# Martinsos/edlib

Measured on AMD Instinct MI355X. Metric: GCUPS (cell updates/s), 1M x 150bp HW reads vs 5Mb target, higher is better.
Workload: dtype u32

## Files before the change

edlib_amd/csrc/engine.hip:

```cpp
#include "engine.hpp"
#include "flat_results.hpp"
#include <sched.h>

#if defined(__x86_64__)
#include <immintrin.h>
#endif
#include <algorithm>
#include <chrono>
#include <atomic>
#include <cmath>
#include <cstdarg>
#include <cstring>
#include <condition_variable>
#include <mutex>
#include <system_error>
#include <thread>

namespace edlib_amd {


static void build_eq8(std::vector<uint8_t>& eq8, const EdlibEqualityPair* eqs, int neq) {
    eq8.assign(256 * 256, 0);
    for (int a = 0; a < 256; ++a) eq8[a * 256 + a] = 1;
    for (int i = 0; i < neq; ++i) {
// ... 16 lines not shown
        const int miss = _mm_movemask_epi8(_mm_cmpeq_epi8(_mm_and_si128(a, b), zero));
        if (miss) return i + __builtin_ctz((unsigned)miss);
    }
    return i;
}
#endif

void build_tables(Tables& tab, const uint8_t* targets, long long totalTargetBytes,
                         const EdlibEqualityPair* eqs, int neq) {
    memset(tab.presence, 0, sizeof tab.presence);
    memset(tab.tlut, 0, sizeof tab.tlut);
    memset(tab.idToByte, 0, sizeof tab.idToByte);
    bool seen[256] = {false};
    tab.sigmaT = 0;
    uint8_t lo[16] = {0}, hi[16] = {0}; int hiBit[16]; int hiBits = 0; bool nibbleOk = true;
    for (int h = 0; h < 16; ++h) hiBit[h] = -1;
#if defined(__x86_64__)
    static const bool haveSsse3 = __builtin_cpu_supports("ssse3");
#else
    static const bool haveSsse3 = false;
#endif
    long long i = 0;
    while (i < totalTargetBytes) {
#if defined(__x86_64__)
        if (haveSsse3 && nibbleOk && tab.sigmaT > 0) {
            i = first_outside_ssse3(targets, i, totalTargetBytes, lo, hi);
            if (i >= totalTargetBytes) break;
        }
#endif
        const uint8_t b = targets[i++];
        if (!seen[b]) {
            seen[b] = true;
            tab.tlut[b] = (uint8_t)tab.sigmaT;
            tab.idToByte[tab.sigmaT] = b;
            tab.presence[b >> 5] |= 1u << (b & 31);
            ++tab.sigmaT;
            if (hiBit[b >> 4] < 0) { if (hiBits < 8) hiBit[b >> 4] = hiBits++; else nibbleOk = false; }
            if (nibbleOk) { hi[b >> 4] = (uint8_t)(1u << hiBit[b >> 4]); lo[b & 15] |= (uint8_t)(1u << hiBit[b >> 4]); }
        }
    }
    tab.eq8.clear();
    if (neq > 0) build_eq8(tab.eq8, eqs, neq);
    for (int q = 0; q < 256; ++q) {
        uint16_t mask = 0;
        for (int s = 0; s < tab.sigmaT && s < 16; ++s)
            if (tab.eq8.empty() ? (q == tab.idToByte[s]) : (tab.eq8[q * 256 + tab.idToByte[s]] != 0)) mask |= (uint16_t)(1u << s);
        tab.eqtbl[q] = mask;
    }
}


__global__ void __launch_bounds__(256)
alphabet_count_kernel(const uint8_t* __restrict__ qpool, const long long* __restrict__ qoff,
                      const uint8_t* __restrict__ tpool, const long long* __restrict__ toff,
                      int shared, const uint32_t* __restrict__ basePresence,
                      const int* __restrict__ unitIdx, int* __restrict__ out)
{
    __shared__ uint32_t s_seen[256];
    s_seen[threadIdx.x] = 0u;
    __syncthreads();
    const int u = unitIdx[blockIdx.x];
    auto scan = [&](const uint8_t* pool, long long lo, long long hi) {
        for (long long c = (lo >> 4) + threadIdx.x; (c << 4) < hi; c += 256) {
            const uint4 v = *reinterpret_cast<const uint4*>(pool + (c << 4));
            const uint32_t d[4] = {v.x, v.y, v.z, v.w};
            const long long at = c << 4;
            if (at >= lo && at + 16 <= hi) {
#pragma unroll
                for (int k = 0; k < 16; ++k) s_seen[(d[k >> 2] >> (8 * (k & 3))) & 0xffu] = 1u;
            } else {
#pragma unroll
                for (int k = 0; k < 16; ++k)
                    if (at + k >= lo && at + k < hi) s_seen[(d[k >> 2] >> (8 * (k & 3))) & 0xffu] = 1u;
            }
        }
    };
    scan(qpool, qoff[u], qoff[u + 1]);
    if (!shared) scan(tpool, toff[u], toff[u + 1]);
    __syncthreads();
    bool present = s_seen[threadIdx.x] != 0u;
    if (shared) present = present || ((basePresence[threadIdx.x >> 5] >> (threadIdx.x & 31)) & 1u);
    const int n = __syncthreads_count(present ? 1 : 0);
    if (threadIdx.x == 0) out[blockIdx.x] = n;
}

__global__ void __launch_bounds__(256)
alphabet_count_short_kernel(const uint8_t* __restrict__ qpool, const long long* __restrict__ qoff,
                            const uint8_t* __restrict__ tpool, const long long* __restrict__ toff,
                            int shared, const uint32_t* __restrict__ basePresence,
                            const int* __restrict__ unitIdx, int n, int* __restrict__ out)
{
    __shared__ uint32_t s_seen[4][64];
    const int lane = threadIdx.x & 63, wv = threadIdx.x >> 6;
    const int slot = blockIdx.x * 4 + wv;
    if (slot >= n) return;
    uint8_t* const seen = reinterpret_cast<uint8_t*>(s_seen[wv]);
    s_seen[wv][lane] = 0u;
    const int u = unitIdx[slot];
    auto scan = [&](const uint8_t* pool, long long lo, long long hi) {
        for (long long c = (lo >> 4) + lane; (c << 4) < hi; c += 64) {
            const uint4 v = *reinterpret_cast<const uint4*>(pool + (c << 4));
            const uint32_t d[4] = {v.x, v.y, v.z, v.w};
            const long long at = c << 4;
#pragma unroll
            for (int k = 0; k < 16; ++k)
                if (at + k >= lo && at + k < hi) seen[(d[k >> 2] >> (8 * (k & 3))) & 0xffu] = 1;
        }
    };
    scan(qpool, qoff[u], qoff[u + 1]);
    if (!shared) scan(tpool, toff[u], toff[u + 1]);
    __builtin_amdgcn_fence(__ATOMIC_RELEASE, "wavefront");
    __builtin_amdgcn_wave_barrier();
    uint32_t w = s_seen[wv][lane];
    if (shared) {
        const uint32_t bits = (basePresence[lane >> 3] >> (4 * (lane & 7))) & 0xfu;
        w |= (bits & 1u) | ((bits & 2u) << 7) | ((bits & 4u) << 14) | ((bits & 8u) << 21);
    }
    int cnt = ((w & 0xffu) != 0) + ((w & 0xff00u) != 0) + ((w & 0xff0000u) != 0) + ((w & 0xff000000u) != 0);
#pragma unroll
    for (int off = 32; off >= 1; off >>= 1) cnt += __shfl_xor(cnt, off, 64);
    if (lane == 0) out[slot] = cnt;
}


Batch::~Batch() {
    DeviceGuard guard(device_);
    if (side_) { (void)hipStreamSynchronize(side_); pool_stream_release(side_); }
    if (aux_) { (void)hipStreamSynchronize(aux_); (void)hipStreamDestroy(aux_); }
    if (stream_) { (void)hipStreamSynchronize(stream_); pool_stream_release(stream_); }
    wideGateRelease();
    for (auto& p : scanEvents_) { pool_event_release(p.first, device_); pool_event_release(p.second, device_); }
}

int roundup(int x, int q) { return (x + q - 1) / q * q; }

int Batch::init(const char* queries, const long long* qoff, int n, const char* targets,
                const long long* toff, int numTargets, EdlibAlignConfig cfg, int device, bool bothStrands, bool hits)
{
    if (n < 0 || (numTargets != 1 && numTargets != n)) { set_error("bad batch shape"); return 1; }
    if (hits) {
        if (numTargets != 1 || bothStrands) { set_error("hit-list read batch: one shared target, one strand"); return 1; }
        if (cfg.mode != EDLIB_MODE_HW) { set_error("hit-list read batch: config.mode must be EDLIB_MODE_HW (SHW and NW have no hit list)"); return 1; }
        if (cfg.task != EDLIB_TASK_DISTANCE) {
            set_error("hit-list read batch: config.task must be EDLIB_TASK_DISTANCE (start locations and paths: align the chosen windows with a pair batch)");
            return 1;
        }
        if (cfg.k < 0) { set_error("hit-list read batch: config.k must be >= 0 (got %d)", cfg.k); return 1; }
        for (int u = 0; u < n; ++u)
            if (qoff[u + 1] - qoff[u] > 32LL * kMaxReadWords) {
                set_error("hit-list read batch: read %d has %lld bases, the limit is %d", u, qoff[u + 1] - qoff[u], 32 * kMaxReadWords);
                return 1;
            }
        bool seen[256] = {false};
        int sigma = 0;
        for (long long j = toff[0]; j < toff[1]; ++j) if (!seen[(uint8_t)targets[j]]) { seen[(uint8_t)targets[j]] = true; ++sigma; }
        if (sigma > 16) { set_error("hit-list read batch: the target has %d distinct symbols, the limit is 16", sigma); return 1; }
    }
    hits_ = hits;
    if (bothStrands && (numTargets != 1 || n > 0x3fffffff)) { set_error("bad both-strand batch shape"); return 1; }
    if (check_device(device)) return 1;
    keep_config(cfg, cfg_, eqs_);
    device_ = device;
    strands_ = bothStrands;
    shared_ = (numTargets == 1);
    if (copy_offsets(qoff, n, "query", qoff_)) return 1;
    const int numReads = n;
    const long long qb = qoff[0];
    if (strands_) {
        n = 2 * numReads;
        qoff_.resize((size_t)n + 1);
        for (int i = 0; i < numReads; ++i) { qoff_[2 * i] = 2 * (qoff[i] - qb); qoff_[2 * i + 1] = 2 * (qoff[i] - qb) + (qoff[i + 1] - qoff[i]); }
        qoff_[n] = 2 * (qoff[numReads] - qb);
    }
    n_ = n;
    if (copy_offsets(toff, numTargets, "target", toff_)) return 1;
    const long long qbytes = qoff_[n] - qoff_[0], tbytes = toff_[numTargets] - toff_[0];
    build_tables(tab_, reinterpret_cast<const uint8_t*>(targets) + toff_[0], tbytes,
                 eqs_.data(), (int)eqs_.size());

    pool_quarantine(false);
    DeviceGuard guard(device_);
    EDLIB_AMD_HIP(guard.status);
    EDLIB_AMD_HIP(pool_stream(&stream_));
    EDLIB_AMD_HIP(evRun0_.create()); EDLIB_AMD_HIP(evRun1_.create());

    const long long tb = toff_[0];
    if (!strands_) for (auto& v : qoff_) v -= qb;
    for (auto& v : toff_) v -= tb;
    {
        const bool inlineT = qbytes + tbytes <= (1 << 20), inlineQ = inlineT && !strands_;
        size_t at = 0;
        auto take = [&](size_t bytes) { const size_t o = at; at = (at + bytes + 15) & ~(size_t)15; return o; };
        const size_t oQoff = take(qoff_.size() * sizeof(long long)), oToff = take(toff_.size() * sizeof(long long));
        const size_t oTlut = take(256), oId = take(256), oEq4 = take(512), oPres = take(32);
        const size_t oQ = inlineQ ? take((size_t)qbytes + 16) : 0, oT = inlineT ? take((size_t)tbytes + 16) : 0;
        EDLIB_AMD_HIP(d_in_.alloc(at));
        EDLIB_AMD_HIP(h_in_.alloc(at));
        uint8_t* h = h_in_.p;
        memcpy(h + oQoff, qoff_.data(), qoff_.size() * sizeof(long long));
        memcpy(h + oToff, toff_.data(), toff_.size() * sizeof(long long));
        memcpy(h + oTlut, tab_.tlut, 256); memcpy(h + oId, tab_.idToByte, 256);
        memcpy(h + oEq4, tab_.eqtbl, 512); memcpy(h + oPres, tab_.presence, 32);
        d_qoff_.alias(d_in_.p + oQoff, qoff_.size()); d_toff_.alias(d_in_.p + oToff, toff_.size());
        d_tlut_.alias(d_in_.p + oTlut, 256); d_idToByte_.alias(d_in_.p + oId, 256);
        d_eqtbl_.alias(d_in_.p + oEq4, 256); d_presence_.alias(d_in_.p + oPres, 8);
        if (inlineQ) {
            if (qbytes) memcpy(h + oQ, queries + qb, (size_t)qbytes);
            memset(h + oQ + qbytes, 0, 16);
            d_qpool_.alias(d_in_.p + oQ, (size_t)qbytes + 16);
        } else {
            EDLIB_AMD_HIP(d_qpool_.alloc((size_t)qbytes + 16));
            if (qbytes && !strands_) EDLIB_AMD_HIP(hipMemcpy(d_qpool_.p, queries + qb, (size_t)qbytes, hipMemcpyHostToDevice));
        }
        if (inlineT) {
            if (tbytes) memcpy(h + oT, targets + tb, (size_t)tbytes);
            memset(h + oT + tbytes, 0, 16);
            d_tpool_.alias(d_in_.p + oT, (size_t)tbytes + 16);
        } else {
            EDLIB_AMD_HIP(d_tpool_.alloc((size_t)tbytes + 16));
            if (tbytes) EDLIB_AMD_HIP(hipMemcpy(d_tpool_.p, targets + tb, (size_t)tbytes, hipMemcpyHostToDevice));
        }
        EDLIB_AMD_HIP(hipMemcpyAsync(d_in_.p, h, at, hipMemcpyHostToDevice, stream_));
    }
    if (strands_) {
        const size_t inBytes = (size_t)(qbytes / 2);
        DevBuf<uint8_t> d_raw;
        EDLIB_AMD_HIP(d_raw.alloc(inBytes + 16));
        if (inBytes) EDLIB_AMD_HIP(hipMemcpy(d_raw.p, queries + qb, inBytes, hipMemcpyHostToDevice));
        EDLIB_AMD_HIP(hipMemsetAsync(d_qpool_.p, 0, (size_t)qbytes + 16, stream_));
        EDLIB_AMD_HIP(launch_strand_pool(d_raw.p, d_qoff_.p, numReads, d_qpool_.p, stream_));
        EDLIB_AMD_HIP(hipStreamSynchronize(stream_));
        EDLIB_AMD_HIP(h_strand_.alloc(2 * (size_t)numReads));
        memset(h_strand_.p, 0, 2 * (size_t)numReads);
    }

    const int mode = (int)cfg_.mode;
    const int modeIn = (int)cfg.mode;
    const bool readsOk = shared_ && tlen(0) > 0 && (tab_.sigmaT <= 4 || (tab_.sigmaT <= 16 && modeIn == EDLIB_MODE_HW));
    syms_ = peq_syms(tab_.sigmaT);
    banded_ = mode == EDLIB_MODE_HW;
    static const int filterFrom = [] {
        const char* e = getenv("EDLIB_AMD_FILTER");
        if (!e || !e[0]) return kFilterFromWords;
        const int v = atoi(e);
        return v <= 0 ? 0 : std::max(kMaxReadWords + 1, std::min(v, kMaxLongReadWords4 + 1));
    }();
    const bool filter = filterFrom > 0 && readsOk && banded_ && modeIn == EDLIB_MODE_HW;
    int groupWords = kMaxReadWords;
    if (banded_ && modeIn == EDLIB_MODE_HW && syms_ <= 8)
        for (int w : {10, 12, 14, 16, 24, 32})
            if (w <= (syms_ == 4 ? kMaxLongReadWords4 : kMaxLongReadWords) && (!filter || w < filterFrom)) groupWords = w;
    const int maxReadLen = 32 * groupWords;
    std::vector<std::vector<int>> byWords(kMaxLongReadWords4 + 1);
    for (int u = 0; u < n; ++u) {
        const int m = qlen(u), T = tlen(u);
        if (m == 0 || T == 0) emptyUnits_.push_back(u);
        else if (readsOk && m <= maxReadLen) { readUnits_.push_back(u); byWords[read_group_words(m)].push_back(u); }
        else if (filter) longUnits_.push_back(u);
        else pairUnits_.push_back(u);
    }
    stats.cells = 0;
    for (int u = 0; u < n; ++u) stats.cells += (long long)qlen(u) * tlen(u);
    {
        alphaUnits_ = emptyUnits_;
        alphaUnits_.insert(alphaUnits_.end(), pairUnits_.begin(), pairUnits_.end());
        alphaUnits_.insert(alphaUnits_.end(), longUnits_.begin(), longUnits_.end());
        long long total = 0;
        for (int u : alphaUnits_) total += qlen(u) + (shared_ ? 0 : tlen(u));
        alphaOnHost_ = h_in_.p && d_qpool_.p && !d_qpool_.owned && total <= 65536;
        alphaBytes_ = total;
    }

    for (int w = 1; w <= kMaxLongReadWords4; ++w) {
        if (byWords[w].empty()) continue;
        std::unique_ptr<ReadGroup> g;
        if (makeGroup(byWords[w], w, g)) return 1;
        if (strands_) {
            for (int sl = 0; sl < g->nslots; sl += 2)
                if (g->perm[sl] >= 0 && ((g->perm[sl] & 1) || g->perm[sl + 1] != g->perm[sl] + 1)) { set_error("both strands: mates are not in adjacent slots"); return 1; }
            g->mates = true;
            EDLIB_AMD_HIP(g->d_win.alloc((size_t)g->nslots / 2));
        }
        groups_.push_back(std::move(g));
    }
    if (initFlatPairs()) return 1;
    const int T = shared_ ? tlen(0) : 0;
    if (!groups_.empty() || !longUnits_.empty()) {
        EDLIB_AMD_HIP(d_tpk_.alloc((size_t)(T + 15) / 16 + 4));
        EDLIB_AMD_HIP(hipMemsetAsync(d_tpk_.p, 0, d_tpk_.bytes(), stream_));
        EDLIB_AMD_HIP(d_wordSteps_.alloc(1));
        EDLIB_AMD_HIP(d_trows_.alloc(((size_t)(T + 15) / 16 + 2) * 8));
    }
    return 0;
}

int Batch::makeGroup(const std::vector<int>& units, int w, std::unique_ptr<ReadGroup>& g, long long oneRoundWaves)
{
    const int mode = (int)cfg_.mode;
    const int T = shared_ ? tlen(0) : 0;
    g.reset(new ReadGroup);
    g->nwords = w;
    g->nslots = roundup((int)units.size(), 64);
    g->perm.assign(g->nslots, -1);
    g->mMin = 0x7fffffff;
    for (int u : units) g->mMin = std::min(g->mMin, qlen(u));
    std::copy(units.begin(), units.end(), g->perm.begin());
    const int nrblk = g->nslots / 64;
    if (mode == EDLIB_MODE_HW) {
        const long long wantWaves = 131072;
        g->warm = 2 * 32 * w - 1;
        long long S = (wantWaves + nrblk - 1) / nrblk;
        const long long maxS = std::max<long long>(1, std::min<long long>(std::min(65535, std::max(1, T / 4096)), T / (4LL * g->warm)));
        S = std::max(1LL, std::min(S, maxS));
        if (oneRoundWaves > 0 && oneRoundWaves / nrblk >= 1) S = std::min(S, oneRoundWaves / nrblk);
        g->segLen = roundup((int)((T + S - 1) / S), 16);
        g->numSegments = (T + g->segLen - 1) / g->segLen;
    } else {
        g->numSegments = 1; g->segLen = roundup(T, 16); g->warm = 0;
    }
    const size_t ns = (size_t)g->nslots, S = (size_t)g->numSegments;
    EDLIB_AMD_HIP(g->d_perm.alloc(ns));
    EDLIB_AMD_HIP(hipMemcpyAsync(g->d_perm.p, g->perm.data(), ns * sizeof(int), hipMemcpyHostToDevice, stream_));
    EDLIB_AMD_HIP(g->d_qlen.alloc(ns)); EDLIB_AMD_HIP(g->d_kinit.alloc(ns));
    g->zeroCopy = ns <= 1024 && pool_enabled();
    if (g->zeroCopy) {
        EDLIB_AMD_HIP(g->hostOut.alloc((ns * 20 + ns + 1) * sizeof(int)));
        int* h = reinterpret_cast<int*>(g->hostOut.p);
        memset(h, 0, (ns * 20 + ns + 1) * sizeof(int));
        g->d_best.alias(h, ns); g->d_total.alias(h + ns, ns); g->d_alphaExtra.alias(h + 2 * ns, ns);
        g->d_flags.alias(h + 3 * ns, ns + 1); g->d_pos.alias(h + 4 * ns + 1, ns * 16);
    } else
    EDLIB_AMD_HIP(g->d_alphaExtra.alloc(ns));
    EDLIB_AMD_HIP(g->d_peq.alloc(ns * (size_t)syms_ * w));
    EDLIB_AMD_HIP(g->d_segBest.alloc(ns * S)); EDLIB_AMD_HIP(g->d_segCnt.alloc(ns * S));
    EDLIB_AMD_HIP(g->d_segPos.alloc(ns * S * 8));
    if (!g->zeroCopy) {
        EDLIB_AMD_HIP(g->d_best.alloc(ns)); EDLIB_AMD_HIP(g->d_total.alloc(ns));
        EDLIB_AMD_HIP(g->d_pos.alloc(ns * 16)); EDLIB_AMD_HIP(g->d_flags.alloc(ns + 1));
    }
    return 0;
}

hipError_t Batch::uploadEq8() {
    if (tab_.eq8.empty() || d_eq8_.p) return hipSuccess;
    hipError_t e = d_eq8_.alloc(65536);
    if (e != hipSuccess) return e;
    return hipMemcpyAsync(d_eq8_.p, tab_.eq8.data(), 65536, hipMemcpyHostToDevice, stream_);
}


void Batch::scanTimerStart() {
    if (scanEventsUsed_ == scanEvents_.size()) {
        hipEvent_t a = nullptr, b = nullptr; int dev = 0;
        (void)pool_event(&a, &dev); (void)pool_event(&b, &dev);
        scanEvents_.push_back({a, b});
    }
    (void)hipEventRecord(scanEvents_[scanEventsUsed_].first, stream_);
}
void Batch::scanTimerStop() {
    (void)hipEventRecord(scanEvents_[scanEventsUsed_].second, stream_);
    ++scanEventsUsed_;
    ++stats.scan_launches;
}


void finalize_semiglobal(UnitResult& r, int kcfg, int m, int best, const int* pos, long long npos) {
    const int W = ((m + 63) / 64) * 64 - m;
    const bool kAllowsM = (kcfg < 0 || kcfg >= m);
    r.ends.clear();
    if (best < 0) {
        if (W > 0 && kAllowsM) { r.editDistance = m; r.ends.push_back(-1); r.hasEnds = true; }
        else { r.editDistance = -1; r.hasEnds = false; }
        return;
    }
    r.editDistance = best;
    r.hasEnds = true;
    if (W > 0 && best == m) r.ends.push_back(-1);
    r.ends.append(pos, (size_t)npos);
}

void blank_record(UnitResult& r) {
    r.status = EDLIB_STATUS_OK; r.editDistance = -1; r.alphabetLength = 0;
    r.hasEnds = r.hasStarts = r.hasAlignment = false;
    r.ends.clear(); r.starts.clear(); r.opsView = nullptr; r.opsViewLen = 0;
}

void finalize_global(UnitResult& r, int kcfg, int mode, int T, int score) {
    if (kcfg >= 0 && score > kcfg) { r.editDistance = -1; r.hasEnds = false; return; }
    r.editDistance = score;
    if (mode == EDLIB_MODE_NW) { r.hasEnds = true; r.ends.assign(1, T - 1); }
    else r.hasEnds = false;
}

int Batch::alphabetBuffers()
{
    const size_t n = alphaUnits_.size();
    if (!side_) EDLIB_AMD_HIP(pool_stream(&side_));
    EDLIB_AMD_HIP(evA_.create());
    if (!d_alphaIdx_.p) {
        EDLIB_AMD_HIP(d_alphaIdx_.alloc(n)); EDLIB_AMD_HIP(d_alphaOut_.alloc(n)); EDLIB_AMD_HIP(alphaPin_.alloc(n * sizeof(int)));
        EDLIB_AMD_HIP(hipMemcpyAsync(d_alphaIdx_.p, alphaUnits_.data(), n * sizeof(int), hipMemcpyHostToDevice, side_));
    }
    return 0;
}

int Batch::alphabetLengthsBegin(hipEvent_t after)
{
    alphaPending_ = false;
    if (alphaUnits_.empty() || alphaOnHost_) return 0;
    const size_t n = alphaUnits_.size();
    if (alphabetBuffers()) return 1;
    EDLIB_AMD_HIP(hipEventRecord(evA_.e, stream_));
    EDLIB_AMD_HIP(hipStreamWaitEvent(side_, evA_.e, 0));
    if (after) EDLIB_AMD_HIP(hipStreamWaitEvent(side_, after, 0));
    if (alphaBytes_ <= 4096LL * (long long)n)
        hipLaunchKernelGGL(alphabet_count_short_kernel, dim3((unsigned)((n + 3) / 4)), dim3(256), 0, side_,
                           d_qpool_.p, d_qoff_.p, d_tpool_.p, d_toff_.p, shared_ ? 1 : 0, d_presence_.p,
                           d_alphaIdx_.p, (int)n, d_alphaOut_.p);
    else
    hipLaunchKernelGGL(alphabet_count_kernel, dim3((unsigned)n), dim3(256), 0, side_,
                       d_qpool_.p, d_qoff_.p, d_tpool_.p, d_toff_.p, shared_ ? 1 : 0, d_presence_.p,
                       d_alphaIdx_.p, d_alphaOut_.p);
    EDLIB_AMD_HIP(hipGetLastError());
    EDLIB_AMD_HIP(evB_.create());
    EDLIB_AMD_HIP(hipEventRecord(evB_.e, side_));
    EDLIB_AMD_HIP(hipMemcpyAsync(alphaPin_.p, d_alphaOut_.p, n * sizeof(int), hipMemcpyDeviceToHost, side_));
    alphaPending_ = true;
    return 0;
}

int Batch::alphabetLengthsEnd(std::vector<UnitResult>& res)
{
    if (alphaUnits_.empty()) return 0;
    if (alphaOnHost_) {
        const uint8_t* hq = h_in_.p + (d_qpool_.p - d_in_.p);
        const uint8_t* ht = h_in_.p + (d_tpool_.p - d_in_.p);
        for (int u : alphaUnits_) {
            bool seen[256] = {false};
            int cnt = 0;
            auto add = [&](const uint8_t* p, long long len) { for (long long i = 0; i < len; ++i) if (!seen[p[i]]) { seen[p[i]] = true; ++cnt; } };
            add(hq + qoff_[u], qlen(u));
            if (!shared_) add(ht + toff_[u], tlen(u));
            else for (int b = 0; b < 256; ++b) if ((tab_.presence[b >> 5] >> (b & 31)) & 1u) { if (!seen[b]) { seen[b] = true; ++cnt; } }
            res[u].alphabetLength = cnt;
        }
        return 0;
    }
    if (!alphaPending_) return 0;
    EDLIB_AMD_HIP(hipStreamSynchronize(side_));
    alphaPending_ = false;
    const int* out = reinterpret_cast<const int*>(alphaPin_.p);
    for (size_t i = 0; i < alphaUnits_.size(); ++i) res[alphaUnits_[i]].alphabetLength = out[i];
    return 0;
}



int Batch::run()
{
    const int rc = runImpl();
    if (rc && wideGateHeld_) {
        if (stream_) { DeviceGuard guard(device_); (void)hipStreamSynchronize(stream_); (void)hipGetLastError(); }
        wideGateRelease();
    }
    return rc;
}

int Batch::beginRun(hipError_t guardStatus)
{
    EDLIB_AMD_HIP(guardStatus);
    const long long cells = stats.cells;
    stats = EdlibAmdBatchStats{};
    stats.cells = cells;
    scanEventsUsed_ = 0;
    wordStepsPending_ = false;
    EDLIB_AMD_HIP(hipEventRecord(evRun0_.e, stream_));
    return 0;
}

int Batch::enqueueWordSteps()
{
    EDLIB_AMD_HIP(h_wordSteps_.alloc(sizeof(unsigned long long)));
    EDLIB_AMD_HIP(hipMemcpyAsync(h_wordSteps_.p, d_wordSteps_.p, sizeof(unsigned long long), hipMemcpyDeviceToHost, stream_));
    wordStepsPending_ = true;
    return 0;
}

int Batch::endRun()
{
    EDLIB_AMD_HIP(hipEventRecord(evRun1_.e, stream_));
    EDLIB_AMD_HIP(hipStreamSynchronize(stream_));
    float ms = 0;
    EDLIB_AMD_HIP(hipEventElapsedTime(&ms, evRun0_.e, evRun1_.e));
    stats.run_ms = ms;
    if (wordStepsPending_) { stats.word_steps += (long long)*reinterpret_cast<unsigned long long*>(h_wordSteps_.p); wordStepsPending_ = false; }
    for (size_t i = 0; i < scanEventsUsed_; ++i) {
        float t = 0;
        EDLIB_AMD_HIP(hipEventElapsedTime(&t, scanEvents_[i].first, scanEvents_[i].second));
        stats.scan_ms += t;
    }
    return 0;
}

int Batch::runImpl()
{
    pool_quarantine(false);
    Lap lap;
    DeviceGuard guard(device_);
    haveResults_ = hitsHaveRun_ = hitList_.result.fetched = false;
    if (beginRun(guard.status)) return 1;
    if (hits_) return runReadHits();
    hostStrandCounts_[0] = hostStrandCounts_[1] = hostStrandCounts_[2] = hostStrandCounts_[3] = 0;
    opsKeep_.clear();
    knownSplits_.clear();
    wideGateRelease();
    wideSerial_ = false;
    viewReady_ = false; cigar_[0].ready = cigar_[1].ready = false; lastRunFlat_ = false;
    opsOwned_.clear();
    std::vector<UnitResult>& res = work_;
    resetRecords(res);
    if (d_ringSteps_.p) EDLIB_AMD_HIP(hipMemsetAsync(d_ringSteps_.p, 0, sizeof(unsigned long long), stream_));
    ringStepsUsed_ = false;
    lap("run: reset records");
    answerEmptyUnits(res);
    alphaDeferred_ = !flatPairs_ && cfg_.mode == EDLIB_MODE_NW && cfg_.task == EDLIB_TASK_DISTANCE && pairUnits_.size() >= 8192 &&
                     groups_.empty() && longUnits_.empty();
    if (!alphaDeferred_ && alphabetLengthsBegin()) return 1;
    flatDone_ = false;
    if (flatPairs_ && runFlatPhase(res, lap)) return 1;
    if (packTarget()) return 1;
    if (runReads()) return 1;
    readsCollected_ = groups_.empty();
    lap("run: reads scans");
    if (!readsCollected_ && cfg_.task != EDLIB_TASK_DISTANCE && collectReads(res)) return 1;
    lap("run: collect reads");
    pairNow_ = pairUnits_;
    if (!longUnits_.empty() && runLongReads(res, lap)) return 1;
    if (banded_ && (!groups_.empty() || !longUnits_.empty()) && enqueueWordSteps()) return 1;
    if (flatDone_) pairNow_.clear();
    if (!pairNow_.empty() && runPairPhase(res, lap)) return 1;
    lap("run: finalize pairs");
    if (!flatDone_ && alphabetLengthsEnd(res)) return 1;
    lap("run: phase 1 (distance)");
    if (strands_ && !res.empty() && resolveStrandsOnHost(res)) return 1;
    live_.clear();
    const bool laterPhases = !flatDone_ && (cfg_.task == EDLIB_TASK_LOC || cfg_.task == EDLIB_TASK_PATH);
    if (laterPhases)
        for (int u = 0; u < n_; ++u)
            if (qlen(u) > 0 && tlen(u) > 0 && res[u].editDistance >= 0) live_.push_back(u);
    if (laterPhases && runStartsPhase(res, lap)) return 1;
    lap("run: phase 2 (starts)");
    if (cfg_.task == EDLIB_TASK_PATH && runPathsPhase(res, lap)) return 1;
    lap("run: phase 3 (paths)");
    if (ringStepsUsed_) EDLIB_AMD_HIP(hipMemcpyAsync(h_ringSteps_.p, d_ringSteps_.p, sizeof(unsigned long long), hipMemcpyDeviceToHost, stream_));
    if (endRun()) return 1;
    if (ringStepsUsed_) stats.word_steps += (long long)*reinterpret_cast<unsigned long long*>(h_ringSteps_.p);
    startStats();
    results_.swap(res);
    haveResults_ = true;
    lap("run: stats");
    if (strands_ && lap.on) {
        int c[4];
        if (strandCounts(c)) return 1;
        fprintf(stderr, "[edlib_amd] strands: %d reads, forward %d, reverse %d, both %d, none %d, located %zu\n", outN(), c[0], c[1],
                c[2], c[3], laterPhases ? live_.size() : (size_t)0);
    }
    return 0;
}

void Batch::resetRecords(std::vector<UnitResult>& res)
{
    const bool lazy = (cfg_.task == EDLIB_TASK_DISTANCE && pairUnits_.empty() && longUnits_.empty() && emptyUnits_.empty() && !groups_.empty()) || flatPairs_;
    pairsCollected_ = true;
    deferReset_ = false;
    deferReadsReset_ = false;
    if (lazy) { res.clear(); return; }
    const size_t keep = std::min(res.size(), (size_t)n_);
    res.resize((size_t)n_);
    deferReset_ = emptyUnits_.empty() && groups_.empty() && longUnits_.empty() && !flatPairs_ && pairUnits_.size() == (size_t)n_;
    deferReadsReset_ = !deferReset_ && cfg_.task != EDLIB_TASK_DISTANCE && emptyUnits_.empty() && pairUnits_.empty() &&
                       longUnits_.empty() && !flatPairs_ && readUnits_.size() == (size_t)n_;
    if (!deferReset_ && !deferReadsReset_) for (size_t u = 0; u < keep; ++u) blank_record(res[u]);
}

void Batch::answerEmptyUnits(std::vector<UnitResult>& res)
{
    const int mode = (int)cfg_.mode;
    for (int u : emptyUnits_) {
        UnitResult& r = res[u];
        const int m = qlen(u), T = tlen(u);
        if (mode == EDLIB_MODE_NW) { r.editDistance = std::max(m, T); r.ends.assign(1, T - 1); r.hasEnds = true; }
        else if (mode == EDLIB_MODE_SHW || mode == EDLIB_MODE_HW) { r.editDistance = m; r.ends.assign(1, -1); r.hasEnds = true; }
        else r.status = EDLIB_STATUS_ERROR;
    }
}

int Batch::runFlatPhase(std::vector<UnitResult>& res, Lap& lap)
{
    bool fell = false;
    if (runPairsFlat(fell)) return 1;
    if (fell) {
        res.resize((size_t)n_);
        for (size_t u = 0; u < res.size(); ++u) blank_record(res[u]);
    } else { flatDone_ = true; pairsCollected_ = false; lastRunFlat_ = true; }
    lap("run: flat pairs");
    return 0;
}

// ... 471 lines not shown
```

edlib_amd/csrc/engine.hpp:

```cpp
#pragma once
#include "../../include/edlib_amd.h"
#include "common.hpp"
#include "pair_kernels.hpp"
#include "lanepair.hpp"
#include "reads_kernels.hpp"
#include "cross_kernels.hpp"
#include "window_kernels.hpp"
#include "strands.hpp"

#include <chrono>
#include <deque>
#include <functional>
#include <memory>
#include <vector>

namespace edlib_amd {

struct Tables {
    uint8_t tlut[256];
    uint8_t idToByte[256];
    int sigmaT = 0;
    uint32_t presence[8];
    uint16_t eqtbl[256];
    std::vector<uint8_t> eq8;
};

struct UnitSpec {
    long long qoff; int qlen; int qstep;
    long long toff; int tlen; int tstep;
    int kinit;
    int skip = 0;
    int band = 0;
};

struct SolveOut {
    std::vector<int> score, count, last;
    std::vector<long long> posStart;
    std::vector<int> posFlat;
    std::vector<const uint8_t*> opsPtr;
    std::vector<int> opsLen;
    std::vector<std::shared_ptr<PinBuf>> opsBufs;
    void reset(size_t n) {
        score.assign(n, -1); count.assign(n, 0); last.assign(n, -1);
        posStart.assign(n + 1, 0); posFlat.clear();
        opsPtr.assign(n, nullptr); opsLen.assign(n, 0); opsBufs.clear();
    }
};

struct Assembler {
    struct Pick { const SolveOut* from = nullptr; size_t q = 0; };
    std::vector<Pick> pick;
    explicit Assembler(size_t n) : pick(n) {}
    void take(size_t i, const SolveOut& from, size_t q) { pick[i].from = &from; pick[i].q = q; }
    void write(SolveOut& out) const {
        out.reset(pick.size());
        for (size_t i = 0; i < pick.size(); ++i) {
            if (const SolveOut* p = pick[i].from) {
                const size_t q = pick[i].q;
                out.score[i] = p->score[q]; out.count[i] = p->count[q]; out.last[i] = p->last[q];
                out.posFlat.insert(out.posFlat.end(), p->posFlat.begin() + p->posStart[q], p->posFlat.begin() + p->posStart[q + 1]);
            }
            out.posStart[i + 1] = (long long)out.posFlat.size();
        }
    }
};

struct BandLadder {
    int mode;
    bool (*enter)(const UnitSpec& u, long long& K);
    UnitSpec (*level)(const UnitSpec& u, long long K);
    bool (*final)(const UnitSpec& u, const UnitSpec& level, int score);
};

struct OpsOut {
    const uint8_t* p = nullptr;
    int len = 0;
    std::vector<uint8_t> own;
};

class LocList {
public:
    LocList() = default;
    ~LocList() { delete big_; }
    LocList(const LocList& o) { append(o.data(), o.n_); }
    LocList& operator=(const LocList& o) { if (this != &o) { clear(); append(o.data(), o.n_); } return *this; }
    LocList(LocList&& o) noexcept : n_(o.n_), big_(o.big_) { in_[0] = o.in_[0]; in_[1] = o.in_[1]; o.n_ = 0; o.big_ = nullptr; }
    LocList& operator=(LocList&& o) noexcept {
        if (this != &o) { delete big_; n_ = o.n_; big_ = o.big_; in_[0] = o.in_[0]; in_[1] = o.in_[1]; o.n_ = 0; o.big_ = nullptr; }
        return *this;
    }
    size_t size() const { return n_; }
    bool empty() const { return n_ == 0; }
    const int* data() const { return n_ <= kInline ? in_ : big_->data(); }
    int* data() { return n_ <= kInline ? in_ : big_->data(); }
    int operator[](size_t i) const { return data()[i]; }
    int& operator[](size_t i) { return data()[i]; }
    void clear() { n_ = 0; }
    void push_back(int v) { append(&v, 1); }
    void append(const int* p, size_t c) {
        const size_t nn = n_ + c;
        if (nn <= kInline) { for (size_t i = 0; i < c; ++i) in_[n_ + i] = p[i]; }
        else {
            if (!big_) big_ = new std::vector<int>();
            if (n_ <= kInline) big_->assign(in_, in_ + n_);
            big_->insert(big_->end(), p, p + c);
        }
        n_ = (uint32_t)nn;
    }
    void assign(size_t c, int v) {
        n_ = 0;
        if (c <= kInline) { for (size_t i = 0; i < c; ++i) in_[i] = v; }
        else { if (!big_) big_ = new std::vector<int>(); big_->assign(c, v); }
        n_ = (uint32_t)c;
    }
private:
    static const uint32_t kInline = 2;
    uint32_t n_ = 0;
    int in_[kInline];
    std::vector<int>* big_ = nullptr;
};

struct UnitResult {
    int status = EDLIB_STATUS_OK;
    int editDistance = -1;
    int alphabetLength = 0;
    bool hasEnds = false, hasStarts = false, hasAlignment = false;
    LocList ends, starts;
    const uint8_t* opsView = nullptr;
    int opsViewLen = 0;
};

struct Lap;
struct ViewLayout;

class Batch {
public:
    virtual ~Batch();
    int init(const char* queries, const long long* qoff, int n,
             const char* targets, const long long* toff, int numTargets,
             EdlibAlignConfig cfg, int device, bool bothStrands = false,
             bool hits = false);
    int run();
    int runImpl();
    int results(EdlibAlignResult* out);
    int resultsFlat(int* status, int* editDistance, int* numLocations, int* alphabetLength, long long* locOffsets,
                    int** endLocations, int** startLocations, long long* alnOffsets, unsigned char** alignment);
    int resultsView(EdlibAmdResultsView* out);
    int cigarView(int format, const char** chars, const long long** offsets);
    int strandView(EdlibAmdStrandView* out);
    int hitsView(EdlibAmdReadHits* out);
    bool isHits() const { return hits_; }
    EdlibAmdBatchStats stats{};
    void finishStats();

private:
    EdlibAlignConfig cfg_{};
    std::vector<EdlibEqualityPair> eqs_;
    int device_ = 0;
    bool shared_ = false;
    int n_ = 0;
    std::vector<long long> qoff_, toff_;
    bool strands_ = false;
    PinBuf h_strand_;
    int outN() const { return strands_ ? n_ / 2 : n_; }
    int unitOf(int u) const { return strands_ ? 2 * u + h_strand_.p[u] : u; }
    void setStrand(int read, int code) { h_strand_.p[read] = (uint8_t)(code & kStrandReverse); h_strand_.p[outN() + read] = (code & kStrandBoth) ? 1 : 0; }
    int resolveStrandsOnHost(std::vector<UnitResult>& res);
    int hostStrandCounts_[4] = {0, 0, 0, 0};
    int strandCounts(int counts[4]);
    Tables tab_;
    hipStream_t stream_ = nullptr;
    Event evRun0_, evRun1_, evA_, evB_;

    DevBuf<uint8_t> d_in_;
    PinBuf h_in_;
    DevBuf<uint8_t> d_qpool_, d_tpool_, d_tlut_, d_idToByte_, d_eq8_;
    DevBuf<uint16_t> d_eqtbl_;
    hipError_t uploadEq8();
    DevBuf<uint32_t> d_presence_;
    DevBuf<long long> d_qoff_, d_toff_;

    std::vector<int> emptyUnits_, readUnits_, pairUnits_;
    std::vector<int> longUnits_;
    std::vector<int> pairNow_;
    int beginRun(hipError_t guardStatus);
    int enqueueWordSteps();
    int endRun();
    void resetRecords(std::vector<UnitResult>& res);
    void answerEmptyUnits(std::vector<UnitResult>& res);
    int runFlatPhase(std::vector<UnitResult>& res, Lap& lap);
    int runLongReads(std::vector<UnitResult>& res, Lap& lap);
    int runPairPhase(std::vector<UnitResult>& res, Lap& lap);
    int runStartsPhase(std::vector<UnitResult>& res, Lap& lap);
    int runPathsPhase(std::vector<UnitResult>& res, Lap& lap);
    void startStats();
    bool flatDone_ = false;

    struct ReadGroup {
        int nwords = 0, nslots = 0, numSegments = 1, segLen = 0, warm = 0, mMin = 0;
        std::vector<int> perm;
        DevBuf<int> d_perm, d_qlen, d_kinit, d_alphaExtra, d_segBest, d_segCnt, d_segPos;
        DevBuf<int> d_best, d_total, d_pos, d_flags;
        DevBuf<uint32_t> d_peq;
        bool zeroCopy = false; PinBuf hostOut;
        std::vector<int> ovfSlots; std::vector<long long> ovfOff; DevBuf<int> d_ovfPool;
        DevBuf<int> d_lvMap, d_lvBest, d_lvCnt, d_lvPos; std::vector<int> lvMap; int lvS = 0, lvCap = 0; bool lvValid = false;
        DevBuf<int> d_list;
        int nreal = -1;
        bool mates = false; DevBuf<int> d_win;
    };
    static constexpr int kLastLevelCap = 16;
    int listOpenSlots(ReadGroup& g, int kDone, std::vector<int>& out);
    DevBuf<uint8_t> d_selTmp_;
    std::vector<std::unique_ptr<ReadGroup>> groups_;
    DevBuf<uint32_t> d_tpk_, d_trows_;
    DevBuf<unsigned long long> d_wordSteps_;
    PinBuf h_wordSteps_; bool wordStepsPending_ = false;
    DevBuf<unsigned long long> d_ringSteps_; PinBuf h_ringSteps_; bool ringStepsUsed_ = false;
    unsigned long long* ringStepsCounter();
    bool banded_ = false;
    int syms_ = 4;
    int packTarget();
    int runReads();
    int makeGroup(const std::vector<int>& units, int words, std::unique_ptr<ReadGroup>& g, long long oneRoundWaves = 0);
    int runGroupScans(ReadGroup& g, bool fullOnly);
    int runGroupExact(ReadGroup& g);
    int collectGroup(ReadGroup& g, std::vector<UnitResult>& res);
    int seedThreshold(const ReadGroup& g, bool fullOnly) const;
    int buildSeedIndex();
    int runSeedPass(ReadGroup& g, int k);
    DevBuf<uint32_t> d_seedCnt_, d_seedOff_, d_seedPos_;
    DevBuf<uint8_t> d_seedTmp_;
    bool hits_ = false, hitsHaveRun_ = false;
    HitListBuffers hitList_;
    HitRows hostHits_;
    DevBuf<int> d_hitSlotUnit_;
    DevBuf<long long> d_hitTotal_;
    int runReadHits();
    int scanGroupHits(ReadGroup& g, int slotBase);
    int hitsScanBanded(ReadGroup& g, int slotBase, const int* d_slotmap, int nlanes, int numSegments, int segLen, int warm);
    struct Piece { long long off; int len; int thr; };
    int scanPieces(const std::vector<Piece>& pieces, bool filter, std::vector<std::pair<int, int>>* cand,
                   std::vector<uint8_t>* overflow, std::vector<int>* best);
    int solveLongReads(std::vector<UnitResult>& res, std::vector<int>& fallback);
    bool filterScan_ = false;
    struct ChainArgs { const uint32_t* in = nullptr; uint32_t* out = nullptr; const int* src = nullptr; int inLanes = 0, blocks = 0; const int* rowBase = nullptr; };
    ChainArgs chain_;
    int solveTallFull(const std::vector<int>& units, std::vector<UnitResult>& res, std::vector<int>& handBack);
    int collectReads(std::vector<UnitResult>& res);
    bool readsCollected_ = true;
    int scanGroup(ReadGroup& g, int mode, const int* d_slotmap, int nlanes, int kcap, const int* d_kinit,
                  int numSegments, int segLen, int warm, int* segBest, int* segCnt, int* segPos, int cap,
                  const long long* posOff, const int* posCap, bool unbanded = false,
                  unsigned long long* wordSteps = nullptr, const uint32_t* peqDense = nullptr,
                  const int* qlenDense = nullptr, bool peqBottom = false);

    DevBuf<PairDesc> d_descs_;
    DevBuf<unsigned long long> d_peq64_;
    DevBuf<StoreEntry> d_store_;
    DevBuf<int> d_aux_, d_out3_, d_outScore_, d_outCount_, d_outLast_, d_posPool_, d_opsLen_, d_alpha_;
    DevBuf<uint8_t> d_ops_;
    DevBuf<long long> d_opsOff_;
    int solve(int mode, bool wantPositions, bool wantPath, const std::vector<UnitSpec>& units, SolveOut& out,
              int ring = 0, int ringH = 1);
    int solveChunk(int mode, bool wantPositions, bool wantPath, const std::vector<UnitSpec>& units,
                   size_t a, size_t b, SolveOut& out, int ring, int ringH);
    static const int kWide = -1;
    static const int kRing32 = -2;
    bool ring32_fits(const std::vector<UnitSpec>& units, size_t a, size_t b, int G) const;
    DevBuf<unsigned long long> d_wide_; DevBuf<unsigned> d_wabort_; PinBuf h_wabort_;
    int wideCap_ = -1;
    struct WidePlan { int slots = 1; size_t perLaunch = 1; };
    int planWide(int mode, PairDesc* descs, size_t n, WidePlan& plan);
    int launchWide(int mode, const PairScanArgs& a, const PairDesc* hostDescs, size_t n, const WidePlan& plan);
    int checkWide();
    bool wideSerial_ = false;
    bool wideGateHeld_ = false;
    void wideGateRelease();
    int solveWideSplit(const std::vector<UnitSpec>& units, std::vector<int>& out, int ring = 0);
    struct KnownSplit { long long qoff; int m; long long toff; int T; int score; int row, left, right; };
    std::vector<KnownSplit> knownSplits_;
    int solveGlobalDistances(const std::vector<UnitSpec>& units, std::vector<int>& score, std::vector<OpsOut>* paths = nullptr);
    int solveSemiGlobal(int mode, bool wantPositions, const std::vector<UnitSpec>& units, SolveOut& out);
    int solveSemiGlobalUnits(int mode, bool wantPositions, const std::vector<UnitSpec>& units, SolveOut& out);
    int solveBanded(const BandLadder& ladder, bool wantPositions, const std::vector<UnitSpec>& units, SolveOut& out);
    int alphabetLengthsBegin(hipEvent_t after = nullptr);
    bool alphaDeferred_ = false;
    int alphabetLengthsEnd(std::vector<UnitResult>& res);
    std::vector<int> alphaUnits_; bool alphaOnHost_ = false, alphaPending_ = false; long long alphaBytes_ = 0;
    hipStream_t side_ = nullptr;
    DevBuf<int> d_alphaIdx_, d_alphaOut_; PinBuf alphaPin_;
    struct PathPiece { long long qoff; int m; long long toff; int T; int score; };
    int hirschbergLevel(const std::vector<PathPiece>& big, std::vector<int>& splitRow,
                        std::vector<int>& leftScore, std::vector<int>& rightScore);
    int solvePaths(const std::vector<PathPiece>& jobs, std::vector<OpsOut>& opsOut, std::vector<int>& status);
    std::vector<std::shared_ptr<PinBuf>> opsKeep_;
    std::deque<std::vector<uint8_t>> opsOwned_;

    int qlen(int u) const { return (int)(qoff_[u + 1] - qoff_[u]); }
    long long tbase(int u) const { return shared_ ? toff_[0] : toff_[u]; }
    int tlen(int u) const { return shared_ ? (int)(toff_[1] - toff_[0]) : (int)(toff_[u + 1] - toff_[u]); }

    void scanTimerStart();
    void scanTimerStop();
    std::vector<std::pair<hipEvent_t, hipEvent_t>> scanEvents_;
    size_t scanEventsUsed_ = 0;

    std::vector<UnitResult> results_, work_;
    std::vector<UnitSpec> startUnits_; std::vector<std::pair<int, int>> startWhere_; std::vector<int> live_;
    bool haveResults_ = false;
    long long algoBase_ = -1;
    bool algoDirty_ = false;
    std::vector<int> pairSpecsFor_;
    std::vector<UnitSpec> pairSpecs_, selScratch_; std::vector<size_t> whoScratch_; std::vector<int> lvlScratch_, scoreMain_;
    SolveOut soMain_, soLevel_;
    int pairSpecsVersion_ = 0, levelSpecsVersion_ = -1, shapeVersion_ = -1, alphaIsPairsVersion_ = -1;
    bool alphaIsPairs_ = false;
    struct PairShape { size_t minBlocks = 0, maxBlocks = 0; int minLenLo = 0, minLenHi = 0, maxDiff = 0; } shape_;
    long long levelPeqWords_ = 0;
    bool levelAllReady_ = false;
    PinBuf h_levelSpecs_, h_levelScore_;
    DevBuf<LevelSpec> d_levelSpecs_;
    DevBuf<PairDesc> d_descsAll_;
    DevBuf<unsigned long long> d_peqAll_;
    hipStream_t aux_ = nullptr;
    Event evLevelIn_, evLevelPeq_;
    int prepareLevelAll(const std::vector<UnitSpec>& units);
    std::function<void()> whileScanning_;
    int runLevelAll(const std::vector<UnitSpec>& units, int ring, int ringH, int ringBlocks, int cap, int kcap, int nbMax);
    int laneSpecsVersion_ = -1;
    long long lanePlaneWords_ = -1, laneTgtWords_ = 0;
    bool laneReady_ = false;
    PinBuf h_laneUnits_, h_laneScore_;
    DevBuf<lanepair::LaneUnit> d_laneUnits_;
    DevBuf<lanepair::Plane2> d_lanePlanes_;
    DevBuf<lanepair::Tgt2> d_laneTgts_;
    DevBuf<int> d_laneFlags_, d_laneScore_;
    Event evLanePack_;
    int alphabetBuffers();
    int prepareLaneLevel(const std::vector<UnitSpec>& units);
    int runLaneLevel(const std::vector<UnitSpec>& units, double rate, int kcap, int W);
    std::vector<OpsOut> fusedOps_;
    bool flatPairs_ = false, pairsCollected_ = true, lastRunFlat_ = false;
    int flatRing_ = 0;
    long long flatWordSteps_ = 0;
    DevBuf<PairDesc> d_flatDescs_;
    DevBuf<int> d_flatOut3_, d_flatPos_, d_flatCensus_;
    PinBuf h_flatCensus_;
    std::vector<long long> flatPeqOff_;
    std::vector<int> flatOvfUnit_; std::vector<long long> flatOvfOff_; std::vector<int> flatOvfPos_;
    PairDesc flatDesc(int u) const;
    int initFlatPairs();
    int runPairsFlat(bool& fellBack);
    bool flatStarts_ = false, flatPaths_ = false, flatNwStore_ = false;
    int flatMaxBlocks_ = 0;
    size_t flatStartCap_ = 0;
    long long flatRevPeqBase_ = 0, flatOpsTotal_ = 0;
    DevBuf<PairDesc> d_flatRevDescs_, d_flatStartDescs_, d_flatPathDescs_;
    DevBuf<int> d_flatSlotOf_, d_flatStartOut3_, d_flatStartsOut_, d_flatPathOut3_, d_flatOpsLen_;
    DevBuf<long long> d_flatOpsOff_, d_flatStoreBase_;
    DevBuf<uint8_t> d_flatOps_;
    std::vector<long long> flatOpsOffHost_;
    int runFlatStartsAndPaths(bool& fellBack);
    int collectPairsFlat(std::vector<UnitResult>& res);
    bool readsViewOnDevice() const;
    int buildReadsView();
    bool flatRing32_ = false; int flatG32_ = 8, flatMaxWords_ = 0;
    bool deferReadsReset_ = false;
    bool deferReset_ = false;
    std::vector<int> flatChunkStart_;
    DevBuf<uint8_t> d_tsym_;
    DevBuf<uint8_t> d_view_; PinBuf h_view_, h_viewVar_; bool viewReady_ = false;
    EdlibAmdResultsView view_{};
    const uint8_t* viewAlnDev_ = nullptr; const long long* viewAlnOffDev_ = nullptr;
    std::vector<int> viewInts_; std::vector<long long> viewOffs_; std::vector<uint8_t> viewOps_;
    DevBuf<int> d_flatOvfAt_, d_flatOvfPool_; DevBuf<long long> d_flatOvfOff_;
    int buildFlatView();
    int buildHostView();
    int fetchViewHead(const ViewLayout& L, long long capLoc, long long capAln, const char* who, long long& nloc, long long& naln);
    struct CigarOut { bool ready = false; PinBuf chars, offs; std::vector<char> hostChars; std::vector<long long> hostOffs; const char* p = nullptr; const long long* off = nullptr; };
    CigarOut cigar_[2];
    DevBuf<long long> d_cigWork_; DevBuf<char> d_cigChars_, d_cigChars2_;
    bool cigarSticky_ = false;
    Event evView_;
    int enqueueCigars(int f, const uint8_t* aln, const long long* alnOff, size_t cap, hipStream_t st);
    int fetchCigars(int f, hipStream_t st);
    int ensureCollected();
};

int align_one(const char* q, int qn, const char* t, int tn, EdlibAlignConfig cfg, EdlibAlignResult* out);
int align_one_fused(const char* q, int qn, const char* t, int tn, EdlibAlignConfig cfg, EdlibAlignResult* out);

struct Lap {
    bool on; std::chrono::steady_clock::time_point t;
    Lap() : on(getenv("EDLIB_AMD_DEBUG") != nullptr), t(std::chrono::steady_clock::now()) {}
    void operator()(const char* what) {
        if (!on) return;
        const auto n = std::chrono::steady_clock::now();
        fprintf(stderr, "[edlib_amd] %-28s %8.3f ms\n", what, std::chrono::duration<double, std::milli>(n - t).count());
        t = n;
    }
};

static inline bool switched_off(const char* v) { return v && v[0] == '0'; }
const int kMaxDevices = 16;
const int kPosCap = 16;
int peq_row_stride(long long nb);
bool needs_hirschberg(int m, int T);
void blank_record(UnitResult& r);
void finalize_global(UnitResult& r, int kcfg, int mode, int T, int score);
long long hw_band_rows(const UnitSpec& u, long long K);
int roundup(int x, int q);
void plan_segments(int nlanes, int T, int mode, int warmFull, long long wantWaves, int& S, int& segLen, int& warm, int minSegCols = 4096);
inline long long tall_round_waves() { return 1024; }
void finalize_semiglobal(UnitResult& r, int kcfg, int m, int best, const int* pos, long long npos);
void build_tables(Tables& tab, const uint8_t* targets, long long totalTargetBytes, const EdlibEqualityPair* eqs, int neq);
int check_device(int device);
void keep_config(const EdlibAlignConfig& cfg, EdlibAlignConfig& kept, std::vector<EdlibEqualityPair>& eqs);
int copy_offsets(const long long* in, int n, const char* what, std::vector<long long>& out);
inline int peq_syms(int sigmaT) { return sigmaT <= 4 ? 4 : (sigmaT <= 8 ? 8 : 16); }

int device_count();
int host_threads(int cap);
int default_device();

}
```

edlib_amd/csrc/engine_reads.hip:

```cpp
#include "engine.hpp"

#include <algorithm>
#include <chrono>
#include <cmath>
#include <condition_variable>
#include <cstring>
#include <mutex>
#include <thread>

namespace edlib_amd {

__global__ void __launch_bounds__(256)
seed_thresholds_kernel(int* __restrict__ kinit, const int* __restrict__ best, const int* __restrict__ cnt, int n)
{
    const int i = blockIdx.x * blockDim.x + threadIdx.x;
    if (i < n && cnt[i] > 0 && best[i] < kinit[i]) kinit[i] = best[i];
}


int Batch::scanGroup(ReadGroup& g, int mode, const int* d_slotmap, int nlanes, int kcap, const int* d_kinit,
                     int numSegments, int segLen, int warm, int* segBest, int* segCnt, int* segPos, int cap,
                     const long long* posOff, const int* posCap, bool unbanded, unsigned long long* wordSteps,
                     const uint32_t* peqDense, const int* qlenDense, bool peqBottom)
{
    ReadScanArgs a{};
    a.peq = peqDense ? peqDense : g.d_peq.p; a.tpk = d_tpk_.p; a.trows = d_trows_.p; a.targetLength = tlen(0);
    if (mode == EDLIB_MODE_SHW) a.targetLength = (int)std::min<long long>(a.targetLength, 64LL * g.nwords + 1);
    a.qlen = qlenDense ? qlenDense : g.d_qlen.p; a.kinit = d_kinit; a.slotmap = d_slotmap; a.nlanes = nlanes;
    a.numSegments = numSegments; a.segLen = segLen; a.warm = warm;
    a.segBest = segBest; a.segCnt = segCnt; a.segPos = segPos; a.cap = cap;
    a.posOff = posOff; a.posCap = posCap;
    a.kcap = kcap; a.wordSteps = wordSteps ? wordSteps : d_wordSteps_.p;
    a.filter = filterScan_ ? 1 : 0;
    a.bottomAligned = peqBottom ? 1 : 0;
    a.chainIn = chain_.in; a.chainOut = chain_.out; a.chainSrc = chain_.src; a.chainInLanes = chain_.inLanes;
    a.chainBlocks = chain_.blocks; a.rowBase = chain_.rowBase;
    const bool chained = chain_.in != nullptr || chain_.out != nullptr;
    static const bool dbg = getenv("EDLIB_AMD_DEBUG") != nullptr;
    if (dbg) {
        EDLIB_AMD_HIP(hipStreamSynchronize(stream_));
        fprintf(stderr, "[edlib_amd] scanGroup nwords=%d mode=%d nlanes=%d S=%d segLen=%d warm=%d cap=%d kcap=%d slotmap=%p posOff=%p\n",
                g.nwords, mode, nlanes, numSegments, segLen, warm, cap, kcap, (const void*)d_slotmap, (const void*)posOff);
    }
    scanTimerStart();
    const bool longGroup = g.nwords > kMaxReadWords;
    const long long colsScanned = std::min<long long>(a.targetLength, (long long)numSegments * segLen) + (long long)(numSegments - 1) * warm;
    const bool fullHeight = banded_ && mode == EDLIB_MODE_HW && unbanded && (chained || syms_ > 4 || longGroup);
    const bool bandedKernel = !fullHeight && banded_ && mode == EDLIB_MODE_HW && (!unbanded || syms_ > 4 || longGroup);
    if (peqBottom && (fullHeight || bandedKernel)) EDLIB_AMD_HIP(hipErrorInvalidValue);
    if (fullHeight) {
        EDLIB_AMD_HIP(launch_scan_reads_full(g.nwords, syms_, a, stream_));
        stats.word_steps += (long long)((nlanes + 63) / 64 * 64) * g.nwords * colsScanned;
    } else if (bandedKernel) EDLIB_AMD_HIP(launch_scan_reads_banded(g.nwords, syms_, a, stream_));
    else {
        EDLIB_AMD_HIP(launch_scan_reads(g.nwords, mode, a, stream_));
        stats.word_steps += (long long)((nlanes + 63) / 64 * 64) * g.nwords * colsScanned;
    }
    scanTimerStop();
    if (dbg) {
        EDLIB_AMD_HIP(hipStreamSynchronize(stream_));
        fprintf(stderr, "[edlib_amd] scanGroup done\n");
    }
    return 0;
}

void plan_segments(int nlanes, int T, int mode, int warmFull, long long wantWaves,
                          int& S, int& segLen, int& warm, int minSegCols)
{
    S = 1; segLen = roundup(T, 16); warm = 0;
    if (mode != EDLIB_MODE_HW) return;
    const long long nrblk = ((long long)nlanes + 63) / 64;
    long long want = (wantWaves + nrblk - 1) / nrblk;
    want = std::max(1LL, std::min<long long>(want, std::min(65535, std::max(1, T / minSegCols))));
    if (warmFull > 0) want = std::max(1LL, std::min<long long>(want, std::max<long long>(1, T / (4LL * warmFull))));
    segLen = roundup((int)((T + want - 1) / want), 16);
    S = (T + segLen - 1) / segLen;
    warm = warmFull;
}

int Batch::runReads()
{
    if (groups_.empty()) return 0;
    stats.path |= 1;
    bool seed = false;
    for (auto& gp : groups_) seed = seed || seedThreshold(*gp, false) >= 0;
    if (seed && buildSeedIndex()) return 1;
    for (auto& gp : groups_) if (runGroupScans(*gp, false)) return 1;
    const int mode = (cfg_.mode == EDLIB_MODE_HW || cfg_.mode == EDLIB_MODE_SHW) ? (int)cfg_.mode : (int)EDLIB_MODE_NW;
    for (auto& gp : groups_)
        if (gp->mates) EDLIB_AMD_HIP(launch_resolve_strands(gp->d_perm.p, gp->d_best.p, gp->d_total.p, gp->nslots, mode, cfg_.k,
                                                            gp->d_win.p, stream_));
    for (auto& gp : groups_) if (runGroupExact(*gp)) return 1;
    return 0;
}

int Batch::runGroupScans(ReadGroup& g, bool fullOnly)
{
    const int T = tlen(0);
    const int mode = (cfg_.mode == EDLIB_MODE_HW || cfg_.mode == EDLIB_MODE_SHW) ? (int)cfg_.mode : (int)EDLIB_MODE_NW;
    const bool banded = banded_ && mode == EDLIB_MODE_HW;
    const int kNoCap = 0x3fffffff;
    static const bool dbgLadder = getenv("EDLIB_AMD_DEBUG") != nullptr;
    EDLIB_AMD_HIP(launch_build_peq_reads(g.nwords, syms_, d_qpool_.p, d_qoff_.p, g.d_perm.p, g.nslots,
                                         d_eqtbl_.p, d_presence_.p, cfg_.k, g.d_peq.p, g.d_qlen.p,
                                         g.d_kinit.p, g.d_alphaExtra.p, stream_));
    const int kSeed = seedThreshold(g, fullOnly);
    const int kFirstMax = kSeed >= 0 ? kSeed : std::max(8, g.nwords / 2);
    int kFirst = (kSeed >= 0 && cfg_.k >= 0) ? std::min(kSeed, cfg_.k) : kFirstMax;
    bool twoPass = !fullOnly && banded && (cfg_.k < 0 || cfg_.k > kFirst) && 32 * g.nwords > kFirst;
    std::vector<int> ladder;
    g.lvValid = false;
    auto probe_scan = [&](const std::vector<int>& map, int kc, std::vector<int>& bestOut) -> int {
        const int nm = (int)map.size();
        int S2, segLen2, warm2;
        plan_segments(nm, T, mode, g.warm, 16384, S2, segLen2, warm2);
        const size_t items = (size_t)nm * S2;
        DevBuf<int> d_map, d_sb, d_sc;
        EDLIB_AMD_HIP(d_map.alloc(nm)); EDLIB_AMD_HIP(d_sb.alloc(items)); EDLIB_AMD_HIP(d_sc.alloc(items));
        EDLIB_AMD_HIP(hipMemcpyAsync(d_map.p, map.data(), nm * sizeof(int), hipMemcpyHostToDevice, stream_));
        if (scanGroup(g, mode, d_map.p, nm, kc, g.d_kinit.p, S2, segLen2, warm2,
                      d_sb.p, d_sc.p, d_sb.p , 0, nullptr, nullptr)) return 1;
        std::vector<int> cnts(items), bests(items);
        EDLIB_AMD_HIP(hipMemcpyAsync(cnts.data(), d_sc.p, items * sizeof(int), hipMemcpyDeviceToHost, stream_));
        EDLIB_AMD_HIP(hipMemcpyAsync(bests.data(), d_sb.p, items * sizeof(int), hipMemcpyDeviceToHost, stream_));
        EDLIB_AMD_HIP(hipStreamSynchronize(stream_));
        bestOut.assign(nm, -1);
        for (int i = 0; i < nm; ++i) {
            int b = 0x7fffffff;
            for (int sg = 0; sg < S2; ++sg)
                if (cnts[(size_t)i * S2 + sg] > 0) b = std::min(b, bests[(size_t)i * S2 + sg]);
            if (b <= kc) bestOut[i] = b;
        }
        return 0;
    };
    auto price_ladder = [&](const std::vector<int>& sample, size_t nOpen, int nReal) -> int {
        const int kTop = std::min(64, 32 * g.nwords - 1);
        std::vector<int> obest;
        if (probe_scan(sample, kTop, obest)) return 1;
        static const int cand[6] = {12, 16, 24, 32, 48, 64};
        auto words = [&](int t) { return std::min<double>(g.nwords, 1.0 + std::max(0, t - 6) / 8.0); };
        auto frac_le = [&](int t) {
            size_t c = 0;
            for (int b : obest) if (b >= 0 && b <= t) ++c;
            return (double)c / (double)obest.size();
        };
        double bestCost = 1e30; int bestMask = 0;
        for (int mask = 0; mask < 64; ++mask) {
            double cost = 0.0, reach = 1.0; bool ok = true;
            for (int q = 0; q < 6; ++q) {
                if (!((mask >> q) & 1)) continue;
                if (cand[q] <= kFirst || cand[q] > kTop) { ok = false; break; }
                cost += reach * words(cand[q]);
                reach = 1.0 - frac_le(cand[q]);
            }
            if (!ok) continue;
            cost += reach * g.nwords;
            if (cost < bestCost - 1e-9) { bestCost = cost; bestMask = mask; }
        }
        for (int q = 0; q < 6; ++q) if ((bestMask >> q) & 1) ladder.push_back(cand[q]);
        if (dbgLadder) {
            fprintf(stderr, "[edlib_amd] ladder nwords=%d kFirst=%d open=%zu/%d levels:", g.nwords, kFirst, nOpen, nReal);
            for (int t : ladder) fprintf(stderr, " %d(%.2f)", t, frac_le(t));
            fprintf(stderr, " full\n");
        }
        return 0;
    };
    if (twoPass && g.nslots >= 16384 && kSeed < 0) {
        const int np = std::max(512, std::min(2048, g.nslots / 32));
        std::vector<int> probe(np);
        for (int i = 0; i < np; ++i) probe[i] = (int)((long long)i * g.nslots / np);
        std::vector<int> pbest;
        if (probe_scan(probe, kFirst, pbest)) return 1;
        int resolved = 0, real = 0;
        std::vector<int> hist(kFirstMax + 1, 0);
        std::vector<int> open;
        for (int i = 0; i < np; ++i) {
            if (g.perm[probe[i]] < 0) continue;
            ++real;
            if (pbest[i] >= 0) { ++resolved; ++hist[pbest[i]]; }
            else if (i == 0 || probe[i] != probe[i - 1]) open.push_back(probe[i]);
        }
        if (resolved > 0) {
            int acc = 0, kq = kFirstMax;
            for (int d = 0; d <= kFirstMax; ++d) { acc += hist[d]; if (acc * 1000LL >= resolved * 995LL) { kq = d; break; } }
            kFirst = std::max(4, std::min(kFirstMax, kq));
        }
        if (real > 0 && resolved * 10 < real * 3) twoPass = false;
        if (twoPass && (int)open.size() * 10 > real && open.size() >= 32 && price_ladder(open, open.size(), real)) return 1;
    }
    std::vector<int> todo;
    bool haveTodo = false;
    if (kSeed >= 0) {
        if (runSeedPass(g, kFirst)) return 1;
        if (twoPass) {
            if (listOpenSlots(g, kFirst, todo)) return 1;
            haveTodo = true;
            if (g.nreal < 0) { g.nreal = 0; for (int u : g.perm) g.nreal += u >= 0; }
            if (g.nslots >= 16384 && todo.size() * 10 > (size_t)g.nreal && todo.size() >= 32) {
                const size_t nsm = std::min<size_t>(2048, todo.size());
                std::vector<int> sample(nsm);
                for (size_t i = 0; i < nsm; ++i) sample[i] = todo[i * todo.size() / nsm];
                if (price_ladder(sample, todo.size(), g.nreal)) return 1;
            }
        }
    } else {
        if (scanGroup(g, mode, nullptr, g.nslots, twoPass ? kFirst : kNoCap, g.d_kinit.p, g.numSegments, g.segLen,
                      g.warm, g.d_segBest.p, g.d_segCnt.p, g.d_segPos.p, 8, nullptr, nullptr, fullOnly)) return 1;
        const bool chained = chain_.in != nullptr || chain_.out != nullptr;
        EDLIB_AMD_HIP(launch_merge_segments(g.d_segBest.p, g.d_segCnt.p, g.d_segPos.p, g.numSegments, 8,
                                            g.nslots, nullptr, 16, g.d_best.p, g.d_total.p, g.d_pos.p,
                                            g.d_flags.p, stream_, chained ? kOvfRescan : kOvfGatherGroup));
    }
    ladder.push_back(kNoCap);
    int kDone = kFirst;
    for (size_t lv = 0; twoPass && lv < ladder.size(); ++lv) {
        const int kcapL = ladder[lv];
        const bool last = kcapL == kNoCap;
        if (!haveTodo && listOpenSlots(g, kDone, todo)) return 1;
        haveTodo = false;
        if (todo.empty()) break;
        {
            const size_t no = todo.size();
            int S2, segLen2, warm2;
            plan_segments((int)no, T, mode, g.warm, 65536, S2, segLen2, warm2);
            const size_t items = no * (size_t)S2;
            const int capL = last ? kLastLevelCap : 8;
            EDLIB_AMD_HIP(g.d_lvMap.ensure(no)); EDLIB_AMD_HIP(g.d_lvBest.ensure(items)); EDLIB_AMD_HIP(g.d_lvCnt.ensure(items));
            EDLIB_AMD_HIP(g.d_lvPos.ensure(items * capL));
            int *d_map = g.d_lvMap.p, *d_sb = g.d_lvBest.p, *d_sc = g.d_lvCnt.p, *d_sp = g.d_lvPos.p;
            EDLIB_AMD_HIP(hipMemcpyAsync(d_map, todo.data(), no * sizeof(int), hipMemcpyHostToDevice, stream_));
            bool plain = false;
            if (last && no >= 4096) {
                const int np2 = 64;
                std::vector<int> sub(np2);
                for (int i = 0; i < np2; ++i) sub[i] = todo[(size_t)((long long)i * no / np2)];
                int S3, segLen3, warm3;
                plan_segments(np2, T, mode, g.warm, 16384, S3, segLen3, warm3);
                const size_t it3 = (size_t)np2 * S3;
                DevBuf<int> d_m3, d_b3, d_c3, d_p3; DevBuf<unsigned long long> d_ws;
                EDLIB_AMD_HIP(d_m3.alloc(np2)); EDLIB_AMD_HIP(d_b3.alloc(it3)); EDLIB_AMD_HIP(d_c3.alloc(it3));
                EDLIB_AMD_HIP(d_p3.alloc(it3 * 8)); EDLIB_AMD_HIP(d_ws.alloc(1));
                EDLIB_AMD_HIP(hipMemcpyAsync(d_m3.p, sub.data(), np2 * sizeof(int), hipMemcpyHostToDevice, stream_));
                EDLIB_AMD_HIP(hipMemsetAsync(d_ws.p, 0, sizeof(unsigned long long), stream_));
                if (scanGroup(g, mode, d_m3.p, np2, kNoCap, g.d_kinit.p, S3, segLen3, warm3,
                              d_b3.p, d_c3.p, d_p3.p, 8, nullptr, nullptr, false, d_ws.p)) return 1;
                unsigned long long ws = 0;
                EDLIB_AMD_HIP(hipMemcpyAsync(&ws, d_ws.p, sizeof ws, hipMemcpyDeviceToHost, stream_));
                EDLIB_AMD_HIP(hipStreamSynchronize(stream_));
                const double cols = (double)np2 * ((double)T + (double)(S3 - 1) * warm3);
                plain = (double)ws >= 0.85 * g.nwords * cols;
                stats.word_steps += (long long)ws;
            }
            const bool bottom = plain && mode == EDLIB_MODE_HW && syms_ == 4 && g.nwords <= kMaxReadWords &&
                                chain_.in == nullptr && chain_.out == nullptr;
            const size_t no64 = (no + 63) / 64 * 64;
            std::vector<int> perm2(no64, -1);
            for (size_t i = 0; i < no; ++i) perm2[i] = g.perm[todo[i]];
            DevBuf<int> d_perm2, d_qlen2, d_kinit2, d_extra2; DevBuf<uint32_t> d_peq2;
            EDLIB_AMD_HIP(d_perm2.alloc(no64)); EDLIB_AMD_HIP(d_qlen2.alloc(no64)); EDLIB_AMD_HIP(d_kinit2.alloc(no64));
            EDLIB_AMD_HIP(d_extra2.alloc(no64)); EDLIB_AMD_HIP(d_peq2.alloc(no64 * (size_t)syms_ * g.nwords));
            EDLIB_AMD_HIP(hipMemcpyAsync(d_perm2.p, perm2.data(), no64 * sizeof(int), hipMemcpyHostToDevice, stream_));
            EDLIB_AMD_HIP(launch_build_peq_reads(g.nwords, syms_, d_qpool_.p, d_qoff_.p, d_perm2.p, (int)no64,
                                                 d_eqtbl_.p, d_presence_.p, cfg_.k, d_peq2.p, d_qlen2.p,
                                                 d_kinit2.p, d_extra2.p, stream_, bottom));
            const int seedCols = 4096;
            DevBuf<int> d_b0, d_c0, d_p0;
            if (mode == EDLIB_MODE_HW && last && no >= 4096 && S2 > 1 && T >= 16 * seedCols) {
                EDLIB_AMD_HIP(d_b0.alloc(no)); EDLIB_AMD_HIP(d_c0.alloc(no)); EDLIB_AMD_HIP(d_p0.alloc(no * 8));
                if (scanGroup(g, mode, nullptr, (int)no, kcapL, d_kinit2.p, 1, seedCols, 0,
                              d_b0.p, d_c0.p, d_p0.p, 8, nullptr, nullptr, plain, nullptr, d_peq2.p, d_qlen2.p, bottom)) return 1;
                hipLaunchKernelGGL(seed_thresholds_kernel, dim3((unsigned)((no + 255) / 256)), dim3(256), 0, stream_,
                                   d_kinit2.p, d_b0.p, d_c0.p, (int)no);
                EDLIB_AMD_HIP(hipGetLastError());
            }
            if (scanGroup(g, mode, nullptr, (int)no, kcapL, d_kinit2.p, S2, segLen2, warm2,
                          d_sb, d_sc, d_sp, capL, nullptr, nullptr, plain, nullptr, d_peq2.p, d_qlen2.p, bottom)) return 1;
            EDLIB_AMD_HIP(launch_merge_segments(d_sb, d_sc, d_sp, S2, capL, (int)no, d_map, 16,
                                                g.d_best.p, g.d_total.p, g.d_pos.p, g.d_flags.p, stream_,
                                                last ? kOvfGatherLevel : kOvfRescan));
            EDLIB_AMD_HIP(hipStreamSynchronize(stream_));
            if (last) { g.lvValid = true; g.lvS = S2; g.lvCap = capL; g.lvMap.swap(todo); }
            if (dbgLadder) fprintf(stderr, "[edlib_amd] level kcap=%d: %zu slots rescanned (plain=%d)\n", kcapL, no, (int)plain);
        }
        kDone = kcapL;
    }
    return 0;
}

int Batch::listOpenSlots(ReadGroup& g, int kDone, std::vector<int>& out)
{
    size_t tmp = 0;
    EDLIB_AMD_HIP(select_slots_scratch_bytes(g.nslots, &tmp));
    EDLIB_AMD_HIP(d_selTmp_.ensure(tmp));
    EDLIB_AMD_HIP(g.d_list.ensure((size_t)g.nslots + 1));
    int* count = g.d_list.p + g.nslots;
    EDLIB_AMD_HIP(launch_select_open_slots(g.d_perm.p, g.d_total.p, g.d_qlen.p, cfg_.k, kDone, g.nslots, g.d_list.p, count,
                                           d_selTmp_.p, d_selTmp_.bytes(), stream_, g.mates));
    int n = 0;
    EDLIB_AMD_HIP(hipMemcpyAsync(&n, count, sizeof(int), hipMemcpyDeviceToHost, stream_));
    EDLIB_AMD_HIP(hipStreamSynchronize(stream_));
    out.resize((size_t)n);
    if (n > 0) {
        EDLIB_AMD_HIP(hipMemcpyAsync(out.data(), g.d_list.p, (size_t)n * sizeof(int), hipMemcpyDeviceToHost, stream_));
        EDLIB_AMD_HIP(hipStreamSynchronize(stream_));
    }
    return 0;
}


int Batch::seedThreshold(const ReadGroup& g, bool fullOnly) const
{
    const long long T = tlen(0);
    if (fullOnly || !banded_ || cfg_.mode != EDLIB_MODE_HW || syms_ != 4 || cfg_.additionalEqualitiesLength > 0 ||
        g.nwords > kMaxReadWords || chain_.in != nullptr || chain_.out != nullptr)
        return -1;
    if (T < 64LL * 32 * g.nwords || g.nslots < 1024 || (long long)g.nslots * T < (1LL << 30)) return -1;
    int kf = -1;
    for (int k = 16; k >= 0 && kf < 0; --k) {
        const int L = g.mMin / (k + 1);
        if (L >= kSeedQ && (double)(k + 1) * (double)T <= std::ldexp(1.0, 2 * L) / 8.0) kf = k;
    }
    return (kf >= 0 && kf >= std::min(8, cfg_.k >= 0 ? cfg_.k : 8)) ? kf : -1;
}

int Batch::buildSeedIndex()
{
    const int T = tlen(0);
    EDLIB_AMD_HIP(d_seedCnt_.ensure((size_t)kSeedBuckets + 1));
    EDLIB_AMD_HIP(d_seedOff_.ensure((size_t)kSeedBuckets + 1));
    EDLIB_AMD_HIP(d_seedPos_.ensure((size_t)T));
    size_t tmp = 0;
    EDLIB_AMD_HIP(seed_index_scratch_bytes(&tmp));
    EDLIB_AMD_HIP(d_seedTmp_.ensure(tmp));
    scanTimerStart();
    EDLIB_AMD_HIP(launch_build_seed_index(d_tpk_.p, T, d_seedCnt_.p, d_seedOff_.p, d_seedPos_.p, d_seedTmp_.p,
                                          d_seedTmp_.bytes(), stream_));
    scanTimerStop();
    return 0;
}

int Batch::runSeedPass(ReadGroup& g, int k)
{
    const int T = tlen(0);
    DevBuf<int> d_back;
    EDLIB_AMD_HIP(d_back.alloc((size_t)g.nslots + 1));
    int* backCount = d_back.p + g.nslots;
    EDLIB_AMD_HIP(hipMemsetAsync(backCount, 0, sizeof(int), stream_));
    SeedArgs a{};
    a.peq = g.d_peq.p; a.qlen = g.d_qlen.p; a.perm = g.d_perm.p; a.tpk = d_tpk_.p; a.targetLength = T;
    a.seedOff = d_seedOff_.p; a.seedPos = d_seedPos_.p; a.nslots = g.nslots; a.k = k;
    a.best = g.d_best.p; a.total = g.d_total.p; a.pos = g.d_pos.p; a.flags = g.d_flags.p;
    a.backSlots = d_back.p; a.backCount = backCount; a.wordSteps = d_wordSteps_.p;
    scanTimerStart();
    EDLIB_AMD_HIP(launch_seed_verify(g.nwords, a, stream_));
    scanTimerStop();
    int nb = 0;
    EDLIB_AMD_HIP(hipMemcpyAsync(&nb, backCount, sizeof(int), hipMemcpyDeviceToHost, stream_));
    EDLIB_AMD_HIP(hipStreamSynchronize(stream_));
    static const bool dbg = getenv("EDLIB_AMD_DEBUG") != nullptr;
    if (dbg) fprintf(stderr, "[edlib_amd] seed pass nwords=%d k=%d: %d of %d slots handed back\n", g.nwords, k, nb, g.nslots);
    if (nb <= 0) return 0;
    int S2, segLen2, warm2;
    plan_segments(nb, T, EDLIB_MODE_HW, g.warm, 65536, S2, segLen2, warm2);
    const size_t items = (size_t)nb * S2;
    DevBuf<int> d_sb, d_sc, d_sp;
    EDLIB_AMD_HIP(d_sb.alloc(items)); EDLIB_AMD_HIP(d_sc.alloc(items)); EDLIB_AMD_HIP(d_sp.alloc(items * 8));
    if (scanGroup(g, EDLIB_MODE_HW, d_back.p, nb, k, g.d_kinit.p, S2, segLen2, warm2, d_sb.p, d_sc.p, d_sp.p, 8,
                  nullptr, nullptr)) return 1;
    EDLIB_AMD_HIP(launch_merge_segments(d_sb.p, d_sc.p, d_sp.p, S2, 8, nb, d_back.p, 16, g.d_best.p, g.d_total.p,
                                        g.d_pos.p, g.d_flags.p, stream_));
    EDLIB_AMD_HIP(hipStreamSynchronize(stream_));
    return 0;
}

int Batch::runGroupExact(ReadGroup& g)
{
    const int T = tlen(0);
    const int mode = (cfg_.mode == EDLIB_MODE_HW || cfg_.mode == EDLIB_MODE_SHW) ? (int)cfg_.mode : (int)EDLIB_MODE_NW;
    const int kNoCap = 0x3fffffff;
    const size_t ns = (size_t)g.nslots;
    g.ovfSlots.clear(); g.ovfOff.assign(1, 0);
    if (mode == EDLIB_MODE_NW) return 0;
    std::vector<int> recs;
    if (g.zeroCopy && !g.mates) {
        EDLIB_AMD_HIP(hipStreamSynchronize(stream_));
        for (size_t s = 0; s < ns; ++s)
            if (g.d_flags.p[s] && g.perm[s] >= 0) { recs.push_back((int)s); recs.push_back(g.d_flags.p[s]); recs.push_back(g.d_total.p[s]); }
    } else {
        size_t tmp = 0;
        EDLIB_AMD_HIP(select_slots_scratch_bytes(g.nslots, &tmp));
        EDLIB_AMD_HIP(d_selTmp_.ensure(tmp));
        EDLIB_AMD_HIP(g.d_list.ensure(ns + 1));
        int* count = g.d_list.p + ns;
        EDLIB_AMD_HIP(launch_select_flagged_slots(g.d_perm.p, g.d_flags.p, g.nslots, g.d_list.p, count,
                                                  d_selTmp_.p, d_selTmp_.bytes(), stream_, g.mates ? g.d_win.p : nullptr));
        int novf = 0;
        EDLIB_AMD_HIP(hipMemcpyAsync(&novf, count, sizeof(int), hipMemcpyDeviceToHost, stream_));
        EDLIB_AMD_HIP(hipStreamSynchronize(stream_));
        if (novf > 0) {
            DevBuf<int> d_recs;
            EDLIB_AMD_HIP(d_recs.alloc((size_t)novf * 3));
            EDLIB_AMD_HIP(launch_pick_slot_records(g.d_list.p, novf, g.d_flags.p, g.d_total.p, d_recs.p, stream_));
            recs.resize((size_t)novf * 3);
            EDLIB_AMD_HIP(hipMemcpyAsync(recs.data(), d_recs.p, recs.size() * sizeof(int), hipMemcpyDeviceToHost, stream_));
            EDLIB_AMD_HIP(hipStreamSynchronize(stream_));
        }
    }
    const size_t no = recs.size() / 3;
    if (!no) return 0;
    std::vector<int> src(no, 0), at(no, -1);
    std::vector<int> rescan;
    for (size_t i = 0; i < no; ++i) {
        const int s = recs[3 * i], f = recs[3 * i + 1];
        g.ovfSlots.push_back(s);
        if (f == kOvfGatherLevel && g.lvValid) {
            const auto it = std::lower_bound(g.lvMap.begin(), g.lvMap.end(), s);
            if (it != g.lvMap.end() && *it == s) { src[i] = 1; at[i] = (int)(it - g.lvMap.begin()); }
        } else if (f == kOvfGatherGroup) { src[i] = 2; at[i] = s; }
        if (!src[i]) { at[i] = (int)rescan.size(); rescan.push_back(s); }
    }
    const size_t nr = rescan.size();
    int S2 = 1, segLen2 = 0, warm2 = 0;
    DevBuf<int> d_map, d_caps, d_sb, d_sc; DevBuf<long long> d_off;
    std::vector<int> cnts;
    if (nr) {
        plan_segments((int)nr, T, mode, g.warm, 16384, S2, segLen2, warm2, nr <= 256 ? 1024 : 4096);
        const size_t items = nr * (size_t)S2;
        EDLIB_AMD_HIP(d_map.alloc(nr)); EDLIB_AMD_HIP(d_sb.alloc(items)); EDLIB_AMD_HIP(d_sc.alloc(items));
        EDLIB_AMD_HIP(hipMemcpyAsync(d_map.p, rescan.data(), nr * sizeof(int), hipMemcpyHostToDevice, stream_));
        if (scanGroup(g, mode, d_map.p, (int)nr, kNoCap, g.d_best.p, S2, segLen2, warm2,
                      d_sb.p, d_sc.p, d_sb.p , 0, nullptr, nullptr)) return 1;
        cnts.resize(items);
        EDLIB_AMD_HIP(hipMemcpyAsync(cnts.data(), d_sc.p, items * sizeof(int), hipMemcpyDeviceToHost, stream_));
        EDLIB_AMD_HIP(hipStreamSynchronize(stream_));
    }
    std::vector<long long> offs(nr * (size_t)S2);
    std::vector<int> gIdx[2], gLim[2]; std::vector<long long> gOff[2];
    long long acc = 0;
    g.ovfOff.assign(no + 1, 0);
    for (size_t i = 0; i < no; ++i) {
        if (src[i]) {
            const int w = src[i] - 1, n = std::max(0, recs[3 * i + 2]);
            gIdx[w].push_back(at[i]); gOff[w].push_back(acc); gLim[w].push_back(n);
            acc += n;
        } else {
            const size_t r = (size_t)at[i];
            for (int sg = 0; sg < S2; ++sg) { offs[r * S2 + sg] = acc; acc += cnts[r * S2 + sg]; }
        }
        g.ovfOff[i + 1] = acc;
    }
    EDLIB_AMD_HIP(g.d_ovfPool.ensure((size_t)std::max<long long>(acc, 1)));
    DevBuf<int> d_gi[2], d_gl[2]; DevBuf<long long> d_go[2];
    for (int w = 0; w < 2; ++w) {
        const size_t n = gIdx[w].size();
        if (!n) continue;
        EDLIB_AMD_HIP(d_gi[w].alloc(n)); EDLIB_AMD_HIP(d_gl[w].alloc(n)); EDLIB_AMD_HIP(d_go[w].alloc(n));
        EDLIB_AMD_HIP(hipMemcpyAsync(d_gi[w].p, gIdx[w].data(), n * sizeof(int), hipMemcpyHostToDevice, stream_));
        EDLIB_AMD_HIP(hipMemcpyAsync(d_gl[w].p, gLim[w].data(), n * sizeof(int), hipMemcpyHostToDevice, stream_));
        EDLIB_AMD_HIP(hipMemcpyAsync(d_go[w].p, gOff[w].data(), n * sizeof(long long), hipMemcpyHostToDevice, stream_));
        if (w == 0)
            EDLIB_AMD_HIP(launch_gather_segments(g.d_lvBest.p, g.d_lvCnt.p, g.d_lvPos.p, g.lvS, g.lvCap, (int)n,
                                                 d_gi[w].p, d_go[w].p, d_gl[w].p, g.d_ovfPool.p, stream_));
        else
            EDLIB_AMD_HIP(launch_gather_segments(g.d_segBest.p, g.d_segCnt.p, g.d_segPos.p, g.numSegments, 8, (int)n,
                                                 d_gi[w].p, d_go[w].p, d_gl[w].p, g.d_ovfPool.p, stream_));
    }
    if (nr) {
        const size_t items = nr * (size_t)S2;
        EDLIB_AMD_HIP(d_caps.alloc(items)); EDLIB_AMD_HIP(d_off.alloc(items));
        EDLIB_AMD_HIP(hipMemcpyAsync(d_caps.p, cnts.data(), items * sizeof(int), hipMemcpyHostToDevice, stream_));
        EDLIB_AMD_HIP(hipMemcpyAsync(d_off.p, offs.data(), items * sizeof(long long), hipMemcpyHostToDevice, stream_));
        if (scanGroup(g, mode, d_map.p, (int)nr, kNoCap, g.d_best.p, S2, segLen2, warm2,
                      d_sb.p, d_sc.p, g.d_ovfPool.p, 0, d_off.p, d_caps.p)) return 1;
    }
    EDLIB_AMD_HIP(hipStreamSynchronize(stream_));
    static const bool dbg = getenv("EDLIB_AMD_DEBUG") != nullptr;
    if (dbg) fprintf(stderr, "[edlib_amd] exact pass nwords=%d: %zu gathered, %zu rescanned\n", g.nwords, no - nr, nr);
    stats.overflow_units += (int)no;
    return 0;
}


int Batch::hitsScanBanded(ReadGroup& g, int slotBase, const int* d_slotmap, int nlanes, int numSegments, int segLen, int warm)
{
    ReadScanArgs a{};
    a.peq = g.d_peq.p; a.tpk = d_tpk_.p; a.trows = d_trows_.p; a.targetLength = tlen(0);
    a.qlen = g.d_qlen.p; a.kinit = g.d_kinit.p; a.slotmap = d_slotmap; a.nlanes = nlanes;
    a.numSegments = numSegments; a.segLen = segLen; a.warm = warm;
    a.cap = 1;
    a.kcap = 0x3fffffff; a.wordSteps = d_wordSteps_.p;
    a.hits = hitList_.list(); a.slotBase = slotBase;
    scanTimerStart();
    EDLIB_AMD_HIP(launch_scan_reads_hits(g.nwords, syms_, a, stream_));
    scanTimerStop();
    return 0;
}

int Batch::scanGroupHits(ReadGroup& g, int slotBase)
{
    const int T = tlen(0);
    const int kSeed = seedThreshold(g, false);
    if (kSeed < 0 || cfg_.k > kSeed) return hitsScanBanded(g, slotBase, nullptr, g.nslots, g.numSegments, g.segLen, g.warm);
    DevBuf<int> d_back;
    EDLIB_AMD_HIP(d_back.alloc((size_t)g.nslots + 1));
    int* backCount = d_back.p + g.nslots;
    EDLIB_AMD_HIP(hipMemsetAsync(backCount, 0, sizeof(int), stream_));
    SeedArgs a{};
    a.peq = g.d_peq.p; a.qlen = g.d_qlen.p; a.perm = g.d_perm.p; a.tpk = d_tpk_.p; a.targetLength = T;
    a.seedOff = d_seedOff_.p; a.seedPos = d_seedPos_.p; a.nslots = g.nslots; a.k = cfg_.k;
    a.backSlots = d_back.p; a.backCount = backCount; a.wordSteps = d_wordSteps_.p;
    a.hits = hitList_.list(); a.slotBase = slotBase;
    scanTimerStart();
    EDLIB_AMD_HIP(launch_seed_verify_hits(g.nwords, a, stream_));
    scanTimerStop();
    int nb = 0;
    EDLIB_AMD_HIP(hipMemcpyAsync(&nb, backCount, sizeof(int), hipMemcpyDeviceToHost, stream_));
    EDLIB_AMD_HIP(hipStreamSynchronize(stream_));
    static const bool dbg = getenv("EDLIB_AMD_DEBUG") != nullptr;
    if (dbg) fprintf(stderr, "[edlib_amd] seed hits pass nwords=%d k=%d: %d of %d slots handed back\n", g.nwords, cfg_.k, nb, g.nslots);
    if (nb > 0) {
        int S2, segLen2, warm2;
        plan_segments(nb, T, EDLIB_MODE_HW, g.warm, 65536, S2, segLen2, warm2);
        if (hitsScanBanded(g, slotBase, d_back.p, nb, S2, segLen2, warm2)) return 1;
        EDLIB_AMD_HIP(hipStreamSynchronize(stream_));
    }
    return 0;
}

int Batch::runReadHits()
{
    const int T = tlen(0);
    stats.path |= 1;
    if (!d_hitSlotUnit_.p) {
        std::vector<int> slotUnit;
        for (auto& gp : groups_) slotUnit.insert(slotUnit.end(), gp->perm.begin(), gp->perm.end());
        for (int u : emptyUnits_) {
            if (T > 0 && qlen(u) == 0) {
                hostHits_.key.push_back((unsigned long long)(uint32_t)slotUnit.size() << 32);
                hostHits_.val[0].push_back(T - 1); hostHits_.val[1].push_back(0); hostHits_.val[2].push_back(0); hostHits_.val[3].push_back(T);
            }
            slotUnit.push_back(u);
        }
        EDLIB_AMD_HIP(d_hitSlotUnit_.alloc(slotUnit.size()));
        if (!slotUnit.empty())
            EDLIB_AMD_HIP(hipMemcpy(d_hitSlotUnit_.p, slotUnit.data(), slotUnit.size() * sizeof(int), hipMemcpyHostToDevice));
        EDLIB_AMD_HIP(d_hitTotal_.alloc(1));
        hitList_.configure("hit-list read batch", "runs", 4, 31, false, kReadHitsExtraBytes);
        if (hitList_.size((size_t)n_, std::max<long long>(1LL << 20, n_), stream_)) return 1;
    }
    if (packTarget()) return 1;
    bool seed = false;
    for (auto& gp : groups_) { const int ks = seedThreshold(*gp, false); seed = seed || (ks >= 0 && cfg_.k <= ks); }
    if (seed && buildSeedIndex()) return 1;
    for (auto& gp : groups_)
        EDLIB_AMD_HIP(launch_build_peq_reads(gp->nwords, syms_, d_qpool_.p, d_qoff_.p, gp->d_perm.p, gp->nslots, d_eqtbl_.p,
                                             d_presence_.p, cfg_.k, gp->d_peq.p, gp->d_qlen.p, gp->d_kinit.p,
                                             gp->d_alphaExtra.p, stream_));
// ... 122 lines not shown
```

edlib_amd/csrc/reads_column_asm.hpp:

```cpp
#pragma once

#define RC_HEAD ".p2align 3\n\ts_nop 0\n\t"
#define RC_W_A(i)        "v_and_b32_e64 %[t], %[e" #i "], %[p" #i "]\n\t"
#define RC_W_ADD0(i)     "v_add_co_u32_e64 %[s], %[cy], %[t], %[p" #i "]\n\t"
#define RC_W_ADDC(i)     "v_addc_co_u32_e64 %[s], %[cy], %[t], %[p" #i "], %[cy]\n\t"
#define RC_W_B(i, c)     "v_bitop3_b32 %[xh], %[s], %[e" #i "], %[p" #i "] bitop3:0xde\n\t" \
                         "v_bitop3_b32 %[ph" #c "], %[m" #i "], %[xh], %[p" #i "] bitop3:0xf1\n\t" \
                         "v_and_b32_e64 %[mh" #c "], %[p" #i "], %[xh]\n\t"
#define RC_W_SH(c, p)    "v_alignbit_b32 %[phs], %[ph" #c "], %[ph" #p "], 31\n\t" "v_alignbit_b32 %[mhs], %[mh" #c "], %[mh" #p "], 31\n\t"
#define RC_W_SH_HW(c)    "v_add_u32_e64 %[phs], %[ph" #c "], %[ph" #c "]\n\t" "v_add_u32_e64 %[mhs], %[mh" #c "], %[mh" #c "]\n\t"
#define RC_W_SH_NW(c)    "v_alignbit_b32 %[phs], %[ph" #c "], -1, 31\n\t" "v_alignbit_b32 %[mhs], %[mh" #c "], 0, 31\n\t"
#define RC_W_C(i)        "v_or_b32_e64 %[xv], %[e" #i "], %[m" #i "]\n\t" \
                         "v_bitop3_b32 %[pn" #i "], %[mhs], %[xv], %[phs] bitop3:0xf1\n\t" \
                         "v_and_b32_e64 %[mn" #i "], %[phs], %[xv]\n\t"
#define RC_SCORE(c)      "v_bfe_u32 %[t], %[ph" #c "], %[sh], 1\n\t" "v_bfe_i32 %[s], %[mh" #c "], %[sh], 1\n\t" "v_add3_u32 %[scoreN], %[score], %[t], %[s]\n\t"
#define RC_SCORE_B(c)    "v_lshrrev_b32_e64 %[t], 31, %[ph" #c "]\n\t" "v_ashrrev_i32_e64 %[s], 31, %[mh" #c "]\n\t" \
                         "v_add_u32_e64 %[scoreN], %[score], %[t]\n\t" "v_add_u32_e64 %[scoreN], %[scoreN], %[s]\n\t"
#define RC_WORD0_HW      RC_W_A(0) RC_W_ADD0(0) RC_W_B(0, 0) RC_W_SH_HW(0) RC_W_C(0)
#define RC_WORD0_NW      RC_W_A(0) RC_W_ADD0(0) RC_W_B(0, 0) RC_W_SH_NW(0) RC_W_C(0)
#define RC_WORD(i, c, p) RC_W_A(i) RC_W_ADDC(i) RC_W_B(i, c) RC_W_SH(c, p) RC_W_C(i)
#define RC_OUT_W(i) [pn##i] "=&v"(Pn[i]), [mn##i] "=&v"(Mn[i])
#define RC_IN_W(i) [e##i] "v"(Eq[i]), [p##i] "v"(Pv[i]), [m##i] "v"(Mv[i])
#define RC_REST_1
#define RC_REST_2 RC_REST_1 RC_WORD(1, 1, 0)
#define RC_REST_3 RC_REST_2 RC_WORD(2, 0, 1)
#define RC_REST_4 RC_REST_3 RC_WORD(3, 1, 0)
#define RC_REST_5 RC_REST_4 RC_WORD(4, 0, 1)
#define RC_REST_6 RC_REST_5 RC_WORD(5, 1, 0)
#define RC_REST_7 RC_REST_6 RC_WORD(6, 0, 1)
#define RC_REST_8 RC_REST_7 RC_WORD(7, 1, 0)
#define RC_OUTS_1 RC_OUT_W(0)
#define RC_INS_1 RC_IN_W(0)
#define RC_OUTS_2 RC_OUTS_1, RC_OUT_W(1)
#define RC_INS_2 RC_INS_1, RC_IN_W(1)
#define RC_OUTS_3 RC_OUTS_2, RC_OUT_W(2)
#define RC_INS_3 RC_INS_2, RC_IN_W(2)
#define RC_OUTS_4 RC_OUTS_3, RC_OUT_W(3)
#define RC_INS_4 RC_INS_3, RC_IN_W(3)
#define RC_OUTS_5 RC_OUTS_4, RC_OUT_W(4)
#define RC_INS_5 RC_INS_4, RC_IN_W(4)
#define RC_OUTS_6 RC_OUTS_5, RC_OUT_W(5)
#define RC_INS_6 RC_INS_5, RC_IN_W(5)
#define RC_OUTS_7 RC_OUTS_6, RC_OUT_W(6)
#define RC_INS_7 RC_INS_6, RC_IN_W(6)
#define RC_OUTS_8 RC_OUTS_7, RC_OUT_W(7)
#define RC_INS_8 RC_INS_7, RC_IN_W(7)
#define RC_LAST_1 0
#define RC_LAST_2 1
#define RC_LAST_3 0
#define RC_LAST_4 1
#define RC_LAST_5 0
#define RC_LAST_6 1
#define RC_LAST_7 0
#define RC_LAST_8 1
#define RC_TEMPS [t] "=&v"(t_), [s] "=&v"(s_), [xh] "=&v"(xh_), [ph0] "=&v"(ph0_), [ph1] "=&v"(ph1_), [mh0] "=&v"(mh0_), [mh1] "=&v"(mh1_), [phs] "=&v"(phs_), [mhs] "=&v"(mhs_), [xv] "=&v"(xv_), [cy] "=&s"(cy_)
#define RC_SCORE_X(c) RC_SCORE(c)
#define RC_SCORE_BX(c) RC_SCORE_B(c)
#define RC_COLUMN_ASM(N, WORD0) asm(RC_HEAD WORD0 RC_REST_##N RC_SCORE_X(RC_LAST_##N) : RC_OUTS_##N, [scoreN] "=&v"(scoreN), RC_TEMPS : RC_INS_##N, [score] "v"(score), [sh] "v"(sh))
#define RC_COLUMN_ASM_B(N, WORD0) asm(RC_HEAD WORD0 RC_REST_##N RC_SCORE_BX(RC_LAST_##N) : RC_OUTS_##N, [scoreN] "=&v"(scoreN), RC_TEMPS : RC_INS_##N, [score] "v"(score))
#define RP_P0 "v56"
#define RP_P1 "v57"
#define RP_PP "v[56:57]"
#define RP_M0 "v58"
#define RP_M1 "v59"
#define RP_MM "v[58:59]"
#define RP_CP "v60"
#define RP_CPP "v[60:61]"
#define RP_CM "v62"
#define RP_CMM "v[62:63]"
#define RP_PL "%[phl]"
#define RP_ML "%[mhl]"
#define RP_W_A(i)          "v_and_b32_e64 %[t], %[e" #i "], %[p" #i "]\n\t"
#define RP_W_ADD0(i)       "v_add_co_u32_e64 %[t], %[cy], %[t], %[p" #i "]\n\t"
#define RP_W_ADDC(i)       "v_addc_co_u32_e64 %[t], %[cy], %[t], %[p" #i "], %[cy]\n\t"
#define RP_W_B(i, PH, MH)  "v_bitop3_b32 %[t], %[t], %[e" #i "], %[p" #i "] bitop3:0xde\n\t" \
                           "v_bitop3_b32 " PH ", %[m" #i "], %[t], %[p" #i "] bitop3:0xf1\n\t" \
                           "v_and_b32_e64 " MH ", %[p" #i "], %[t]\n\t"
#define RP_S1_0(PH, MH)    RP_W_A(0) RP_W_ADD0(0) RP_W_B(0, PH, MH)
#define RP_S1(i, PH, MH)   RP_W_A(i) RP_W_ADDC(i) RP_W_B(i, PH, MH)
#define RP_S2(i, PH, MH)   "v_or_b32_e64 %[t], %[e" #i "], %[m" #i "]\n\t" \
                           "v_bitop3_b32 %[pn" #i "], " MH ", %[t], " PH " bitop3:0xf1\n\t" \
                           "v_and_b32_e64 %[mn" #i "], " PH ", %[t]\n\t"
#define RP_CARRY           "v_lshrrev_b32_e64 " RP_CP ", 31, " RP_P1 "\n\t" "v_lshrrev_b32_e64 " RP_CM ", 31, " RP_M1 "\n\t"
#define RP_SHL             "v_lshlrev_b64 " RP_PP ", 1, " RP_PP "\n\t" "v_lshlrev_b64 " RP_MM ", 1, " RP_MM "\n\t"
#define RP_SHLADD          "v_lshl_add_u64 " RP_PP ", " RP_PP ", 1, " RP_CPP "\n\t" "v_lshl_add_u64 " RP_MM ", " RP_MM ", 1, " RP_CMM "\n\t"
#define RP_LONE            "v_alignbit_b32 " RP_PL ", " RP_PL ", " RP_P1 ", 31\n\t" "v_alignbit_b32 " RP_ML ", " RP_ML ", " RP_M1 ", 31\n\t"
#define RP_SCORE(PH, MH)   "v_lshrrev_b32_e64 %[t], 31, " PH "\n\t" "v_add_u32_e64 %[scoreN], %[score], %[t]\n\t" \
                           "v_ashrrev_i32_e64 %[t], 31, " MH "\n\t" "v_add_u32_e64 %[scoreN], %[scoreN], %[t]\n\t"
#define RP_PAIR01          RP_S1_0(RP_P0, RP_M0) RP_S1(1, RP_P1, RP_M1)
#define RP_BODY_2 RP_PAIR01 RP_SCORE(RP_P1, RP_M1) RP_SHL RP_S2(0, RP_P0, RP_M0) RP_S2(1, RP_P1, RP_M1)
#define RP_BODY_3 RP_PAIR01 RP_S1(2, RP_PL, RP_ML) RP_SCORE(RP_PL, RP_ML) RP_LONE RP_SHL \
                  RP_S2(0, RP_P0, RP_M0) RP_S2(1, RP_P1, RP_M1) RP_S2(2, RP_PL, RP_ML)
#define RP_BODY_4 RP_PAIR01 RP_CARRY RP_SHL RP_S2(0, RP_P0, RP_M0) RP_S2(1, RP_P1, RP_M1) \
                  RP_S1(2, RP_P0, RP_M0) RP_S1(3, RP_P1, RP_M1) RP_SCORE(RP_P1, RP_M1) RP_SHLADD RP_S2(2, RP_P0, RP_M0) RP_S2(3, RP_P1, RP_M1)
#define RP_BODY_5 RP_PAIR01 RP_CARRY RP_SHL RP_S2(0, RP_P0, RP_M0) RP_S2(1, RP_P1, RP_M1) \
                  RP_S1(2, RP_P0, RP_M0) RP_S1(3, RP_P1, RP_M1) RP_S1(4, RP_PL, RP_ML) RP_SCORE(RP_PL, RP_ML) RP_LONE RP_SHLADD \
                  RP_S2(2, RP_P0, RP_M0) RP_S2(3, RP_P1, RP_M1) RP_S2(4, RP_PL, RP_ML)
#define RP_TEMPS [t] "=&v"(t_), [ph0] "=&{v56}"(ph0_), [ph1] "=&{v57}"(ph1_), [mh0] "=&{v58}"(mh0_), [mh1] "=&{v59}"(mh1_), [cy] "=&s"(cy_)
#define RP_TEMPS_LONE , [phl] "=&v"(phl_), [mhl] "=&v"(mhl_)
#define RP_TEMPS_CARRY , [cp] "=&{v60}"(cp_), [cm] "=&{v62}"(cm_)
#define RP_INS_CARRY , [z0] "{v61}"(zr0), [z1] "{v63}"(zr1)
#define RP_XT_2
#define RP_XI_2
#define RP_XT_3 RP_TEMPS_LONE
#define RP_XI_3
#define RP_XT_4 RP_TEMPS_CARRY
#define RP_XI_4 RP_INS_CARRY
#define RP_XT_5 RP_TEMPS_LONE RP_TEMPS_CARRY
#define RP_XI_5 RP_INS_CARRY
#define RP_COLUMN_ASM_B(N) asm(RC_HEAD RP_BODY_##N : RC_OUTS_##N, [scoreN] "=&v"(scoreN), RP_TEMPS RP_XT_##N : RC_INS_##N, [score] "v"(score) RP_XI_##N)
#define RP_COLUMN_DISPATCH_B(NWD) \
    if constexpr (NWD == 2) RP_COLUMN_ASM_B(2); if constexpr (NWD == 3) RP_COLUMN_ASM_B(3); \
    if constexpr (NWD == 4) RP_COLUMN_ASM_B(4); if constexpr (NWD == 5) RP_COLUMN_ASM_B(5);
#define RC_COLUMN_ASM_NS(N, WORD0) asm(RC_HEAD WORD0 RC_REST_##N : RC_OUTS_##N, RC_TEMPS : RC_INS_##N)
#define RC_COLUMN_DISPATCH_NS(NA, WORD0) \
    if constexpr (NA == 1) RC_COLUMN_ASM_NS(1, WORD0); if constexpr (NA == 2) RC_COLUMN_ASM_NS(2, WORD0); if constexpr (NA == 3) RC_COLUMN_ASM_NS(3, WORD0); \
    if constexpr (NA == 4) RC_COLUMN_ASM_NS(4, WORD0); if constexpr (NA == 5) RC_COLUMN_ASM_NS(5, WORD0); if constexpr (NA == 6) RC_COLUMN_ASM_NS(6, WORD0); \
    if constexpr (NA == 7) RC_COLUMN_ASM_NS(7, WORD0); if constexpr (NA == 8) RC_COLUMN_ASM_NS(8, WORD0);
#define RC_COLUMN_DISPATCH_B(NWD, WORD0) \
    if constexpr (NWD == 1) RC_COLUMN_ASM_B(1, WORD0); if constexpr (NWD == 2) RC_COLUMN_ASM_B(2, WORD0); if constexpr (NWD == 3) RC_COLUMN_ASM_B(3, WORD0); \
    if constexpr (NWD == 4) RC_COLUMN_ASM_B(4, WORD0); if constexpr (NWD == 5) RC_COLUMN_ASM_B(5, WORD0); if constexpr (NWD == 6) RC_COLUMN_ASM_B(6, WORD0); \
    if constexpr (NWD == 7) RC_COLUMN_ASM_B(7, WORD0); if constexpr (NWD == 8) RC_COLUMN_ASM_B(8, WORD0);
#define RC_COLUMN_DISPATCH(NWD, WORD0) \
    if constexpr (NWD == 1) RC_COLUMN_ASM(1, WORD0); if constexpr (NWD == 2) RC_COLUMN_ASM(2, WORD0); if constexpr (NWD == 3) RC_COLUMN_ASM(3, WORD0); \
    if constexpr (NWD == 4) RC_COLUMN_ASM(4, WORD0); if constexpr (NWD == 5) RC_COLUMN_ASM(5, WORD0); if constexpr (NWD == 6) RC_COLUMN_ASM(6, WORD0); \
    if constexpr (NWD == 7) RC_COLUMN_ASM(7, WORD0); if constexpr (NWD == 8) RC_COLUMN_ASM(8, WORD0);
```

edlib_amd/csrc/reads_kernels.hip:

```cpp
#include "reads_kernels.hpp"
#include "reads_scan.hpp"
#include "reads_column_asm.hpp"

namespace edlib_amd {


__global__ void __launch_bounds__(256)
pack_target_2bit_kernel(const uint8_t* __restrict__ raw, const uint8_t* __restrict__ lut,
                        int T, u32* __restrict__ tpk, int nwords)
{
    __shared__ uint8_t s_lut[256];
    s_lut[threadIdx.x] = lut[threadIdx.x];
    __syncthreads();
    const int w = blockIdx.x * blockDim.x + threadIdx.x;
    if (w >= nwords) return;
    const int base = w * 16;
    u32 out = 0;
    if (base + 16 <= T) {
        const uint4 v = *reinterpret_cast<const uint4*>(raw + base);
        const u32 d[4] = {v.x, v.y, v.z, v.w};
#pragma unroll
        for (int i = 0; i < 16; ++i)
            out |= (u32)(s_lut[(d[i >> 2] >> ((i & 3) * 8)) & 0xFF] & 3) << (2 * i);
    } else {
        for (int i = 0; i < 16 && base + i < T; ++i)
            out |= (u32)(s_lut[raw[base + i]] & 3) << (2 * i);
    }
    tpk[w] = out;
}

__global__ void __launch_bounds__(256)
pack_target_rows_kernel(const uint8_t* __restrict__ raw, const uint8_t* __restrict__ lut, int T,
                        u32* __restrict__ trows, int ndwords)
{
    __shared__ uint8_t s_lut[256];
    s_lut[threadIdx.x] = lut[threadIdx.x];
    __syncthreads();
    const int w = blockIdx.x * blockDim.x + threadIdx.x;
    if (w >= ndwords) return;
    const int c = 2 * w;
    const u32 a0 = c < T ? (u32)(s_lut[raw[c]] & 15) : 0u, a1 = c + 1 < T ? (u32)(s_lut[raw[c + 1]] & 15) : 0u;
    trows[w] = (a0 << 8) | (a1 << 24);
}

hipError_t launch_pack_target_rows(const uint8_t* raw, const uint8_t* lut, int T, u32* trows, int ndwords,
                                   hipStream_t stream)
{
    if (ndwords == 0) return hipSuccess;
    hipLaunchKernelGGL(pack_target_rows_kernel, dim3((ndwords + 255) / 256), dim3(256), 0, stream,
                       raw, lut, T, trows, ndwords);
    return hipGetLastError();
}

hipError_t launch_pack_target_2bit(const uint8_t* raw, const uint8_t* lut, int T, u32* tpk,
                                   hipStream_t stream)
{
    const int nwords = (T + 15) / 16;
    if (nwords == 0) return hipSuccess;
    hipLaunchKernelGGL(pack_target_2bit_kernel, dim3((nwords + 255) / 256), dim3(256), 0, stream,
                       raw, lut, T, tpk, nwords);
    return hipGetLastError();
}


template <int NWD>
__global__ void __launch_bounds__(256)
build_peq_reads_kernel(const uint8_t* __restrict__ reads, const long long* __restrict__ qoff,
                       const int* __restrict__ perm, int nslots, int S,
                       const uint16_t* __restrict__ eqtbl, const u32* __restrict__ tpres, int kcfg,
                       u32* __restrict__ peq, int* __restrict__ qlen, int* __restrict__ kinit,
                       int* __restrict__ alphaExtra, int bottomAlign)
{
    __shared__ uint16_t s_eq[256];
    s_eq[threadIdx.x] = eqtbl[threadIdx.x];
    __syncthreads();
    const int lane = threadIdx.x & 63;
    const int blk = blockIdx.x * 4 + (threadIdx.x >> 6);
    if (blk * 64 >= nslots) return;
    const int slot = blk * 64 + lane;
    const int r = slot < nslots ? perm[slot] : -1;
    long long off = 0; int m = 1;
    if (r >= 0) { off = qoff[r]; m = (int)(qoff[r + 1] - off); }
    int extra = 0;
    for (int g0 = 0; g0 < S; g0 += 4) {
        u32 E[4][NWD];
#pragma unroll
        for (int s = 0; s < 4; ++s)
#pragma unroll
            for (int d = 0; d < NWD; ++d) E[s][d] = 0;
        for (int j = 0; j < 64; ++j) {
            const int rj = __builtin_amdgcn_readlane(r, j);
            if (rj < 0) continue;
            const int mj = __builtin_amdgcn_readlane(m, j);
            const long long offj = ((long long)__builtin_amdgcn_readlane((int)(off >> 32), j) << 32)
                                 | (u32)__builtin_amdgcn_readlane((int)off, j);
            unsigned long long seen0 = 0, seen1 = 0, seen2 = 0, seen3 = 0;
            int extraJ = 0;
            const bool mine = lane == j;
            const int padj = bottomAlign ? 32 * NWD - mj : 0;
#pragma unroll
            for (int c = 0; c < (NWD + 1) / 2; ++c) {
                const int i = 64 * c + lane - padj;
                const bool in = i >= 0 && i < mj;
                const u32 by = in ? reads[offj + i] : 0u;
                const u32 mask = in ? ((u32)s_eq[by] >> g0) : (i < 0 ? 0xfu : 0u);
                const unsigned long long b0 = __builtin_amdgcn_ballot_w64((mask & 1u) != 0), b1 = __builtin_amdgcn_ballot_w64((mask & 2u) != 0);
                const unsigned long long b2 = __builtin_amdgcn_ballot_w64((mask & 4u) != 0), b3 = __builtin_amdgcn_ballot_w64((mask & 8u) != 0);
                constexpr int w0 = 0;
                const int d0 = 2 * c, d1 = (2 * c + 1 < NWD) ? 2 * c + 1 : w0;
                E[0][d0] = (mine ? (u32)b0 : E[0][d0]); E[1][d0] = (mine ? (u32)b1 : E[1][d0]);
                E[2][d0] = (mine ? (u32)b2 : E[2][d0]); E[3][d0] = (mine ? (u32)b3 : E[3][d0]);
                if (2 * c + 1 < NWD) {
                    E[0][d1] = (mine ? (u32)(b0 >> 32) : E[0][d1]); E[1][d1] = (mine ? (u32)(b1 >> 32) : E[1][d1]);
                    E[2][d1] = (mine ? (u32)(b2 >> 32) : E[2][d1]); E[3][d1] = (mine ? (u32)(b3 >> 32) : E[3][d1]);
                }
                if (g0 == 0) {
                    unsigned long long np = __builtin_amdgcn_ballot_w64(in && !((tpres[by >> 5] >> (by & 31)) & 1u));
                    while (np) {
                        const int l = __builtin_ctzll(np);
                        const u32 v = (u32)__builtin_amdgcn_readlane((int)by, l);
                        const unsigned long long bit = 1ull << (v & 63);
                        unsigned long long& sw = (v >> 6) == 0 ? seen0 : (v >> 6) == 1 ? seen1 : (v >> 6) == 2 ? seen2 : seen3;
                        if (!(sw & bit)) { sw |= bit; ++extraJ; }
                        np &= ~__builtin_amdgcn_ballot_w64(in && by == v);
                    }
                }
            }
            if (g0 == 0 && mine) extra = extraJ;
        }
        if (slot < nslots) {
#pragma unroll
            for (int s = 0; s < 4; ++s)
#pragma unroll
                for (int d = 0; d < NWD; ++d)
                    peq[((size_t)(blk * S + g0 + s) * NWD + d) * 64 + lane] = E[s][d];
        }
    }
    if (slot >= nslots) return;
    qlen[slot] = m;
    kinit[slot] = (kcfg < 0 || kcfg > m) ? m : kcfg;
    alphaExtra[slot] = extra;
}

template <int NWD>
static hipError_t launch_build_peq_t(const uint8_t* reads, const long long* qoff, const int* perm,
                                     int nslots, int S, const uint16_t* eqtbl, const u32* tpres, int kcfg,
                                     u32* peq, int* qlen, int* kinit, int* alphaExtra,
                                     hipStream_t stream, bool bottomAlign)
{
    hipLaunchKernelGGL(build_peq_reads_kernel<NWD>, dim3((nslots + 255) / 256), dim3(256), 0, stream,
                       reads, qoff, perm, nslots, S, eqtbl, tpres, kcfg, peq, qlen, kinit, alphaExtra, bottomAlign ? 1 : 0);
    return hipGetLastError();
}

hipError_t launch_build_peq_reads(int nwords, int syms, const uint8_t* reads, const long long* qoff,
                                  const int* perm, int nslots, const uint16_t* eqtbl,
                                  const u32* tpres, int kcfg, u32* peq, int* qlen, int* kinit,
                                  int* alphaExtra, hipStream_t stream, bool bottomAlign)
{
    if (nslots == 0) return hipSuccess;
    if (syms != 4 && syms != 8 && syms != 16) return hipErrorInvalidValue;
    switch (nwords) {
#define CASE(N) case N: return launch_build_peq_t<N>(reads, qoff, perm, nslots, syms, eqtbl, tpres, kcfg, peq, qlen, kinit, alphaExtra, stream, bottomAlign);
        CASE(1) CASE(2) CASE(3) CASE(4) CASE(5) CASE(6) CASE(7) CASE(8) CASE(10) CASE(12) CASE(14) CASE(16) CASE(24) CASE(32)
#undef CASE
    }
    return hipErrorInvalidValue;
}


#define EDLIB_AMD_DISPATCH_COLUMN(sym)                                                     \
    switch (sym) {                                                                         \
        case 0:  column_step<NWD, MODE, BOTTOM>(E0, Pv, Mv, score, sh, zr0, zr1); asm volatile("; sym0"); break; \
        case 1:  column_step<NWD, MODE, BOTTOM>(E1, Pv, Mv, score, sh, zr0, zr1); asm volatile("; sym1"); break; \
        case 2:  column_step<NWD, MODE, BOTTOM>(E2, Pv, Mv, score, sh, zr0, zr1); asm volatile("; sym2"); break; \
        default: column_step<NWD, MODE, BOTTOM>(E3, Pv, Mv, score, sh, zr0, zr1); asm volatile("; sym3"); break; \
    }

#define EDLIB_AMD_TRACK_SCORE(sc, col)                         \
    if ((sc) <= best) {                                        \
        if ((sc) < best) { best = (sc); cnt = 0; }             \
        if (cnt < cap) pos[cnt] = (col);                       \
        ++cnt;                                                 \
    }
#define EDLIB_AMD_TRACK(col) EDLIB_AMD_TRACK_SCORE(score, col)

template <int NWD, int MODE, bool BOTTOM = false>
__global__ void __launch_bounds__(256)
scan_reads_kernel(const ReadScanArgs a)
{
    constexpr int kHitGroup = 4;
    const int lane = threadIdx.x & 63;
    const int rblk = blockIdx.x * 4 + (threadIdx.x >> 6);
    const int seg = blockIdx.y;
    const int idx = rblk * 64 + lane;
    if (rblk * 64 >= a.nlanes) return;
    const bool live = idx < a.nlanes;
    const int slot = live ? (a.slotmap ? a.slotmap[idx] : idx) : 0;

    u32 E0[NWD], E1[NWD], E2[NWD], E3[NWD], Pv[NWD], Mv[NWD];
    {
        const size_t pb = (size_t)(slot >> 6) * 4 * NWD * 64 + (slot & 63);
#pragma unroll
        for (int d = 0; d < NWD; ++d) {
            E0[d] = a.peq[pb + (size_t)(0 * NWD + d) * 64];
            E1[d] = a.peq[pb + (size_t)(1 * NWD + d) * 64];
            E2[d] = a.peq[pb + (size_t)(2 * NWD + d) * 64];
            E3[d] = a.peq[pb + (size_t)(3 * NWD + d) * 64];
            Pv[d] = ~0u;
            Mv[d] = 0u;
        }
    }
    const int m = a.qlen[slot];
    if constexpr (BOTTOM) {
        const int pad = 32 * NWD - m;
#pragma unroll
        for (int d = 0; d < NWD; ++d) {
            const int lo = pad - 32 * d;
            Pv[d] = lo <= 0 ? ~0u : (lo >= 32 ? 0u : ~0u << lo);
        }
    }
    const u32 sh = (u32)(m - 1) & 31u;
    u32 zr0 = 0, zr1 = 0;
    if constexpr (BOTTOM && (NWD == 4 || NWD == 5)) {
        asm volatile("v_mov_b32 %0, 0" : "=v"(zr0));
        asm volatile("v_mov_b32 %0, 0" : "=v"(zr1));
    }
    int score = m;
    int best = a.kinit[slot];
    int cnt = 0;
    const long long item = (long long)idx * a.numSegments + seg;
    const int cap = !live ? 0 : (a.posCap ? a.posCap[item] : a.cap);
    int* pos = a.segPos + (!live ? 0 : (a.posOff ? a.posOff[item] : item * a.cap));

    const int T = a.targetLength;
    const int c0 = seg * a.segLen;
    int c1 = c0 + a.segLen; if (c1 > T) c1 = T;
    int cw = c0 - a.warm; if (cw < 0) cw = 0;
    cw &= ~15;

    for (int w = cw >> 4; w < (c0 >> 4); ++w) {
        const u32 tw = a.tpk[w];
#pragma unroll
        for (int j = 0; j < 16; ++j) {
            const u32 sym = (tw >> (2 * j)) & 3u;
            EDLIB_AMD_DISPATCH_COLUMN(sym)
        }
    }
    const int wend = c1 >> 4;
    int lim = best + (kHitGroup - 1);
    for (int w = c0 >> 4; w < wend; ++w) {
        const u32 tw = a.tpk[w];
#pragma unroll
        for (int j = 0; j < 16; j += kHitGroup) {
            int sc[kHitGroup];
#pragma unroll
            for (int q = 0; q < kHitGroup; ++q) {
                const u32 sym = (tw >> (2 * (j + q))) & 3u;
                EDLIB_AMD_DISPATCH_COLUMN(sym)
                sc[q] = score;
            }
            if (MODE != 0) {
                if (__builtin_expect(score <= lim, 0)) {
                    best = lim - (kHitGroup - 1);
#pragma unroll
                    for (int q = 0; q < kHitGroup; ++q) { EDLIB_AMD_TRACK_SCORE(sc[q], w * 16 + j + q) }
                    lim = best + (kHitGroup - 1);
                }
            }
        }
    }
    best = lim - (kHitGroup - 1);
    const int rem = c1 - (wend << 4);
    if (rem > 0) {
        u32 tw = a.tpk[wend];
        for (int j = 0; j < rem; ++j) {
            const u32 sym = tw & 3u;
            tw >>= 2;
            EDLIB_AMD_DISPATCH_COLUMN(sym)
            if (MODE != 0) { EDLIB_AMD_TRACK(wend * 16 + j) }
        }
    }
    if (live) {
        const size_t o = (size_t)idx * a.numSegments + seg;
        a.segBest[o] = (MODE == 0) ? score : best;
        a.segCnt[o] = (MODE == 0) ? 1 : cnt;
    }
}

template <int NWD>
static hipError_t launch_scan_mode(int mode, const ReadScanArgs& a, hipStream_t stream)
{
    const int nrblk = (a.nlanes + 63) / 64;
    dim3 grid((nrblk + 3) / 4, a.numSegments), block(256);
    switch (mode) {
        case 0: hipLaunchKernelGGL((scan_reads_kernel<NWD, 0>), grid, block, 0, stream, a); break;
        case 1: hipLaunchKernelGGL((scan_reads_kernel<NWD, 1>), grid, block, 0, stream, a); break;
        case 2: if (a.bottomAligned) hipLaunchKernelGGL((scan_reads_kernel<NWD, 2, true>), grid, block, 0, stream, a);
                else hipLaunchKernelGGL((scan_reads_kernel<NWD, 2>), grid, block, 0, stream, a);
                break;
        default: return hipErrorInvalidValue;
    }
    return hipGetLastError();
}

hipError_t launch_scan_reads(int nwords, int mode, const ReadScanArgs& a, hipStream_t stream)
{
    if (a.nlanes == 0) return hipSuccess;
    if (a.bottomAligned && mode != 2) return hipErrorInvalidValue;
    switch (nwords) {
#define CASE(N) case N: return launch_scan_mode<N>(mode, a, stream);
        CASE(1) CASE(2) CASE(3) CASE(4) CASE(5) CASE(6) CASE(7) CASE(8)
#undef CASE
    }
    return hipErrorInvalidValue;
}


hipError_t launch_scan_reads_full_long(int nwords, int syms, const ReadScanArgs& a, hipStream_t stream);
hipError_t launch_scan_reads_banded_long(int nwords, int syms, const ReadScanArgs& a, hipStream_t stream);

template <int S, bool CHAIN>
static hipError_t launch_scan_reads_full_s(int nwords, const ReadScanArgs& a, hipStream_t stream)
{
    dim3 grid((a.nlanes + 63) / 64, a.numSegments), block(64);
    switch (nwords) {
#define CASE(N) case N: EDLIB_AMD_CHECK_STATIC_LDS((scan_reads_full_kernel<N, S, CHAIN>), N * S * 256); \
                        hipLaunchKernelGGL((scan_reads_full_kernel<N, S, CHAIN>), grid, block, 0, stream, a); break;
        CASE(1) CASE(2) CASE(3) CASE(4) CASE(5) CASE(6) CASE(7) CASE(8)
#undef CASE
        default: return hipErrorInvalidValue;
    }
    return hipGetLastError();
}

hipError_t launch_scan_reads_full(int nwords, int syms, const ReadScanArgs& a, hipStream_t stream)
{
    if (a.nlanes == 0) return hipSuccess;
    if (nwords > kMaxReadWords) return launch_scan_reads_full_long(nwords, syms, a, stream);
    const bool chain = a.chainIn != nullptr || a.chainOut != nullptr;
    switch (syms) {
        case 4: return chain ? launch_scan_reads_full_s<4, true>(nwords, a, stream) : launch_scan_reads_full_s<4, false>(nwords, a, stream);
        case 8: return chain ? launch_scan_reads_full_s<8, true>(nwords, a, stream) : launch_scan_reads_full_s<8, false>(nwords, a, stream);
        case 16: return chain ? launch_scan_reads_full_s<16, true>(nwords, a, stream) : launch_scan_reads_full_s<16, false>(nwords, a, stream);
    }
    return hipErrorInvalidValue;
}

template <int S>
static hipError_t launch_scan_reads_banded_s(int nwords, const ReadScanArgs& a, hipStream_t stream)
{
    const int nrblk = (a.nlanes + 63) / 64;
    dim3 grid(nrblk, a.numSegments), block(64);
    switch (nwords) {
#define CASE(N) case N: if (a.filter) { EDLIB_AMD_CHECK_STATIC_LDS((scan_reads_banded_kernel<N, S, true>), N * S * 256); \
                                            hipLaunchKernelGGL((scan_reads_banded_kernel<N, S, true>), grid, block, 0, stream, a); } \
                        else { EDLIB_AMD_CHECK_STATIC_LDS((scan_reads_banded_kernel<N, S, false>), N * S * 256); \
                               hipLaunchKernelGGL((scan_reads_banded_kernel<N, S, false>), grid, block, 0, stream, a); } break;
        CASE(1) CASE(2) CASE(3) CASE(4) CASE(5) CASE(6) CASE(7) CASE(8)
#undef CASE
        default: return hipErrorInvalidValue;
    }
    return hipGetLastError();
}

hipError_t launch_scan_reads_banded(int nwords, int syms, const ReadScanArgs& a, hipStream_t stream)
{
    if (a.nlanes == 0) return hipSuccess;
    if (nwords > kMaxReadWords) return a.filter ? hipErrorInvalidValue : launch_scan_reads_banded_long(nwords, syms, a, stream);
    switch (syms) {
        case 4: return launch_scan_reads_banded_s<4>(nwords, a, stream);
        case 8: return launch_scan_reads_banded_s<8>(nwords, a, stream);
        case 16: return launch_scan_reads_banded_s<16>(nwords, a, stream);
    }
    return hipErrorInvalidValue;
}


__global__ void __launch_bounds__(256)
collect_candidates_kernel(const int* __restrict__ segCnt, const int* __restrict__ segPos, int S, int cap, int nlanes,
                          int* __restrict__ out, int maxOut, int* __restrict__ counter, int* __restrict__ overflow)
{
    const long long item = (long long)blockIdx.x * blockDim.x + threadIdx.x;
    if (item >= (long long)nlanes * S) return;
    const int c = segCnt[item];
    if (c <= 0) return;
    const int lane = (int)(item / S);
    if (c > cap) overflow[lane] = 1;
    const int take = c < cap ? c : cap;
    const int at = atomicAdd(counter, take);
    for (int i = 0; i < take; ++i)
        if (at + i < maxOut) { out[2 * (at + i)] = lane; out[2 * (at + i) + 1] = segPos[item * cap + i]; }
}

hipError_t launch_collect_candidates(const int* segCnt, const int* segPos, int numSegments, int cap, int nlanes,
                                     int* out, int maxOut, int* counter, int* overflow, hipStream_t stream)
{
    const long long items = (long long)nlanes * numSegments;
    if (items == 0) return hipSuccess;
    hipLaunchKernelGGL(collect_candidates_kernel, dim3((unsigned)((items + 255) / 256)), dim3(256), 0, stream,
                       segCnt, segPos, numSegments, cap, nlanes, out, maxOut, counter, overflow);
    return hipGetLastError();
}


__global__ void __launch_bounds__(256)
merge_segments_kernel(const int* __restrict__ segBest, const int* __restrict__ segCnt,
                      const int* __restrict__ segPos, int S, int cap, int nlanes,
                      const int* __restrict__ slotmap, int capFinal,
                      int* __restrict__ best, int* __restrict__ total, int* __restrict__ pos,
                      int* __restrict__ flags, int gatherFlag)
{
    const int idx = blockIdx.x * blockDim.x + threadIdx.x;
    if (idx >= nlanes) return;
    const int slot = slotmap ? slotmap[idx] : idx;
    const size_t base = (size_t)idx * S;
    int b = 0x7fffffff;
    for (int s = 0; s < S; ++s)
        if (segCnt[base + s] > 0 && segBest[base + s] < b) b = segBest[base + s];
    int n = 0, ovf = 0;
    if (b != 0x7fffffff) {
        for (int s = 0; s < S; ++s) {
            const int c = segCnt[base + s];
            if (c <= 0 || segBest[base + s] != b) continue;
            if (c > cap) ovf = 1;
            const int take = c < cap ? c : cap;
            for (int i = 0; i < take; ++i)
                if (n + i < capFinal) pos[(size_t)slot * capFinal + n + i] = segPos[(base + s) * cap + i];
            n += c;
        }
        if (!ovf && n > capFinal) ovf = gatherFlag;
    }
    best[slot] = (b == 0x7fffffff) ? -1 : b;
    total[slot] = n;
    flags[slot] = ovf;
}

__global__ void __launch_bounds__(64)
merge_segments_wave_kernel(const int* __restrict__ segBest, const int* __restrict__ segCnt,
                           const int* __restrict__ segPos, int S, int cap, int nlanes,
                           const int* __restrict__ slotmap, int capFinal,
                           int* __restrict__ best, int* __restrict__ total, int* __restrict__ pos,
                           int* __restrict__ flags, int gatherFlag)
{
    const int idx = blockIdx.x, lane = threadIdx.x;
    const int slot = slotmap ? slotmap[idx] : idx;
    const size_t base = (size_t)idx * S;
    int b = 0x7fffffff;
    for (int s = lane; s < S; s += 64)
        if (segCnt[base + s] > 0 && segBest[base + s] < b) b = segBest[base + s];
    for (int off = 32; off; off >>= 1) { const int o = __shfl_xor(b, off); b = o < b ? o : b; }
    int n = 0, ovf = 0;
    if (b != 0x7fffffff) {
        for (int s0 = 0; s0 < S; s0 += 64) {
            const int s = s0 + lane;
            int c = s < S ? segCnt[base + s] : 0;
            if (c <= 0 || segBest[base + s] != b) c = 0;
            if (c > cap) ovf = 1;
            int incl = c;
            for (int d = 1; d < 64; d <<= 1) { const int t = __shfl_up(incl, d); if (lane >= d) incl += t; }
            const int at = n + incl - c, take = c < cap ? c : cap;
            for (int i = 0; i < take; ++i)
                if (at + i < capFinal) pos[(size_t)slot * capFinal + at + i] = segPos[(base + s) * cap + i];
            n += __shfl(incl, 63);
        }
        ovf = __any(ovf) ? 1 : 0;
        if (!ovf && n > capFinal) ovf = gatherFlag;
    }
    if (lane == 0) {
        best[slot] = (b == 0x7fffffff) ? -1 : b;
        total[slot] = n;
        flags[slot] = ovf;
    }
}

hipError_t launch_merge_segments(const int* segBest, const int* segCnt, const int* segPos, int S,
                                 int cap, int nlanes, const int* slotmap, int capFinal, int* best,
                                 int* total, int* pos, int* flags, hipStream_t stream, int gatherFlag)
{
    if (nlanes == 0) return hipSuccess;
    if (S >= 64) {
        hipLaunchKernelGGL(merge_segments_wave_kernel, dim3(nlanes), dim3(64), 0, stream,
                           segBest, segCnt, segPos, S, cap, nlanes, slotmap, capFinal, best, total, pos, flags, gatherFlag);
        return hipGetLastError();
    }
    hipLaunchKernelGGL(merge_segments_kernel, dim3((nlanes + 255) / 256), dim3(256), 0, stream,
                       segBest, segCnt, segPos, S, cap, nlanes, slotmap, capFinal, best, total, pos, flags, gatherFlag);
    return hipGetLastError();
}

__global__ void __launch_bounds__(64)
gather_segments_kernel(const int* __restrict__ segBest, const int* __restrict__ segCnt,
                       const int* __restrict__ segPos, int S, int cap, const int* __restrict__ idx,
                       const long long* __restrict__ off, const int* __restrict__ lim, int* __restrict__ out)
{
    const int lane = threadIdx.x;
    const size_t base = (size_t)idx[blockIdx.x] * S;
    int* dst = out + off[blockIdx.x];
    const int capOut = lim[blockIdx.x];
    int b = 0x7fffffff;
    for (int s = lane; s < S; s += 64)
        if (segCnt[base + s] > 0 && segBest[base + s] < b) b = segBest[base + s];
    for (int o = 32; o; o >>= 1) { const int t = __shfl_xor(b, o); b = t < b ? t : b; }
    if (b == 0x7fffffff) return;
    int n = 0;
    for (int s0 = 0; s0 < S; s0 += 64) {
        const int s = s0 + lane;
        int c = s < S ? segCnt[base + s] : 0;
        if (c <= 0 || segBest[base + s] != b) c = 0;
        int incl = c;
        for (int d = 1; d < 64; d <<= 1) { const int t = __shfl_up(incl, d); if (lane >= d) incl += t; }
        const int at = n + incl - c, take = c < cap ? c : cap;
        for (int i = 0; i < take; ++i)
            if (at + i < capOut) dst[at + i] = segPos[(base + s) * cap + i];
        n += __shfl(incl, 63);
    }
}

hipError_t launch_gather_segments(const int* segBest, const int* segCnt, const int* segPos, int S, int cap, int n,
                                  const int* idx, const long long* off, const int* lim, int* out, hipStream_t stream)
{
    if (n == 0) return hipSuccess;
    hipLaunchKernelGGL(gather_segments_kernel, dim3(n), dim3(64), 0, stream, segBest, segCnt, segPos, S, cap, idx, off, lim, out);
    return hipGetLastError();
}

}
```

edlib_amd/csrc/reads_kernels.hpp:

```cpp
#pragma once
#include <hip/hip_runtime.h>
#include <stdint.h>

#include "hit_list.hpp"

namespace edlib_amd {

constexpr int kMaxReadWords = 8;
constexpr int kMaxLongReadWords = 16;
constexpr int kMaxLongReadWords4 = 32;
constexpr int kFilterFromWords = 13;
inline int read_group_words(int m) { const int w = (m + 31) / 32; return w <= kMaxReadWords ? w : (w <= 10 ? 10 : (w <= 12 ? 12 : (w <= 14 ? 14 : (w <= 16 ? 16 : (w <= 24 ? 24 : 32))))); }
constexpr int kLanes = 64;


struct ReadScanArgs {
    const uint32_t* peq;
    const uint32_t* tpk;
    const uint32_t* trows;
    int targetLength;
    const int* qlen;
    const int* kinit;
    const int* slotmap;
    int nlanes;
    int numSegments;
    int segLen;
    int warm;
    int* segBest;
    int* segCnt;
    int* segPos;
    int cap;
    const long long* posOff;
    const int* posCap;
    int kcap;
    unsigned long long* wordSteps;
    const uint32_t* chainIn; uint32_t* chainOut;
    const int* chainSrc;
    int chainInLanes;
    int chainBlocks;
    const int* rowBase;
    int filter;
    HitList hits;
    int slotBase;
    int bottomAligned;
};

hipError_t launch_scan_reads(int nwords, int mode, const ReadScanArgs& a, hipStream_t stream);

hipError_t launch_scan_reads_banded(int nwords, int syms, const ReadScanArgs& a, hipStream_t stream);

hipError_t launch_scan_reads_full(int nwords, int syms, const ReadScanArgs& a, hipStream_t stream);

hipError_t launch_pack_target_2bit(const uint8_t* raw, const uint8_t* lut, int targetLength,
                                   uint32_t* tpk, hipStream_t stream);
hipError_t launch_pack_target_rows(const uint8_t* raw, const uint8_t* lut, int targetLength,
                                   uint32_t* trows, int ndwords, hipStream_t stream);

hipError_t launch_build_peq_reads(int nwords, int syms, const uint8_t* reads, const long long* qoff,
                                  const int* perm, int nslots, const uint16_t* eqtbl,
                                  const uint32_t* targetPresence , int kcfg,
                                  uint32_t* peq, int* qlen, int* kinit, int* alphaExtra,
                                  hipStream_t stream, bool bottomAlign = false);

hipError_t launch_collect_candidates(const int* segCnt, const int* segPos, int numSegments, int cap, int nlanes,
                                     int* out, int maxOut, int* counter, int* overflow, hipStream_t stream);

constexpr int kSeedQ = 12;
constexpr int kSeedBuckets = 1 << (2 * kSeedQ);
constexpr int kSeedBucketCap = 64;
constexpr int kSeedMaxDiag = 32;
constexpr int kSeedMaxWindow = 1024;

struct SeedArgs {
    const uint32_t* peq;
    const int* qlen;
    const int* perm;
    const uint32_t* tpk;
    int targetLength;
    const uint32_t* seedOff;
    const uint32_t* seedPos;
    int nslots;
    int k;
    int* best; int* total; int* pos; int* flags;
    int* backSlots; int* backCount;
    unsigned long long* wordSteps;
    HitList hits;
    int slotBase;
};

hipError_t seed_index_scratch_bytes(size_t* bytes);
hipError_t launch_build_seed_index(const uint32_t* tpk, int targetLength, uint32_t* cnt, uint32_t* off, uint32_t* pos,
                                   void* tmp, size_t tmpBytes, hipStream_t stream);
hipError_t launch_seed_verify(int nwords, const SeedArgs& a, hipStream_t stream);

hipError_t launch_merge_segments(const int* segBest, const int* segCnt, const int* segPos,
                                 int numSegments, int cap, int nlanes, const int* slotmap, int capFinal,
                                 int* best, int* total, int* pos, int* flags, hipStream_t stream, int gatherFlag = 1);
constexpr int kOvfRescan = 1, kOvfGatherLevel = 2, kOvfGatherGroup = 4;
hipError_t launch_gather_segments(const int* segBest, const int* segCnt, const int* segPos, int numSegments, int cap, int n,
                                  const int* idx, const long long* off, const int* lim, int* out, hipStream_t stream);

hipError_t select_slots_scratch_bytes(int nslots, size_t* bytes);
hipError_t launch_select_open_slots(const int* perm, const int* total, const int* qlen, int kcfg, int kDone, int nslots,
                                    int* out, int* count, void* tmp, size_t tmpBytes, hipStream_t stream, bool mates = false);
hipError_t launch_select_flagged_slots(const int* perm, const int* flags, int nslots, int* out, int* count,
                                       void* tmp, size_t tmpBytes, hipStream_t stream, const int* win = nullptr);
hipError_t launch_pick_slot_records(const int* slots, int n, const int* flags, const int* total, int* out, hipStream_t stream);

hipError_t launch_scan_reads_hits(int nwords, int syms, const ReadScanArgs& a, hipStream_t stream);
hipError_t launch_seed_verify_hits(int nwords, const SeedArgs& a, hipStream_t stream);
constexpr int kReadHitsExtraBytes = 12;
hipError_t launch_read_hits_finish(HitListBuffers& hl, const int* slotUnit, int numUnits, long long* total, hipStream_t stream);

}
```

edlib_amd/csrc/reads_scan.hpp:

```cpp
#pragma once
#include "lds_check.hpp"
#include "reads_kernels.hpp"
#include "reads_column_asm.hpp"

namespace edlib_amd {

typedef uint32_t u32;


template <int NWD, int MODE, bool BOTTOM = false>
__device__ __forceinline__ void column_step(const u32 (&Eq)[NWD], u32 (&Pv)[NWD], u32 (&Mv)[NWD],
                                            int& score, const u32 sh, const u32 zr0 = 0, const u32 zr1 = 0)
{
    static_assert(!BOTTOM || (MODE == 2 && NWD <= 8), "bottom-aligned rows: HW, up to 8 words");
    if constexpr (BOTTOM && NWD >= 2 && NWD <= 5) {
        u32 t_, ph0_, ph1_, mh0_, mh1_, phl_, mhl_, cp_, cm_, Pn[NWD], Mn[NWD];
        int scoreN;
        unsigned long long cy_;
        RP_COLUMN_DISPATCH_B(NWD)
#pragma unroll
        for (int i = 0; i < NWD; ++i) { Pv[i] = Pn[i]; Mv[i] = Mn[i]; }
        score = scoreN;
        return;
    } else if constexpr (BOTTOM) {
        u32 t_, s_, xh_, ph0_, ph1_, mh0_, mh1_, phs_, mhs_, xv_, Pn[NWD], Mn[NWD];
        int scoreN;
        unsigned long long cy_;
        RC_COLUMN_DISPATCH_B(NWD, RC_WORD0_HW)
#pragma unroll
        for (int i = 0; i < NWD; ++i) { Pv[i] = Pn[i]; Mv[i] = Mn[i]; }
        score = scoreN;
        return;
    } else if constexpr (NWD <= 8) {
        u32 t_, s_, xh_, ph0_, ph1_, mh0_, mh1_, phs_, mhs_, xv_, Pn[NWD], Mn[NWD];
        int scoreN;
        unsigned long long cy_;
        if constexpr (MODE == 2) { RC_COLUMN_DISPATCH(NWD, RC_WORD0_HW) } else { RC_COLUMN_DISPATCH(NWD, RC_WORD0_NW) }
#pragma unroll
        for (int i = 0; i < NWD; ++i) { Pv[i] = Pn[i]; Mv[i] = Mn[i]; }
        score = scoreN;
        return;
    }
    u32 Ph[NWD], Mh[NWD];
    u32 carry = 0;
#pragma unroll
    for (int i = 0; i < NWD; ++i) {
        const u32 t = Eq[i] & Pv[i];
        u32 cout;
        const u32 s = __builtin_addc(t, Pv[i], carry, &cout);
        carry = cout;
        const u32 Xh = (s ^ Pv[i]) | Eq[i];
        Ph[i] = Mv[i] | ~(Xh | Pv[i]);
        Mh[i] = Pv[i] & Xh;
    }
    score += (int)__builtin_amdgcn_ubfe(Ph[NWD - 1], sh, 1) + __builtin_amdgcn_sbfe(Mh[NWD - 1], sh, 1);
#pragma unroll
    for (int i = NWD - 1; i >= 0; --i) {
        u32 ph, mh;
        if (i > 0) {
            ph = __builtin_amdgcn_alignbit(Ph[i], Ph[i - 1], 31);
            mh = __builtin_amdgcn_alignbit(Mh[i], Mh[i - 1], 31);
        } else {
            ph = (Ph[0] << 1) | (MODE == 2 ? 0u : 1u);
            mh = Mh[0] << 1;
        }
        const u32 Xv = Eq[i] | Mv[i];
        Pv[i] = mh | ~(Xv | ph);
        Mv[i] = ph & Xv;
    }
}


#define BITOP3_XOR_OR(a, b, c)   __builtin_amdgcn_bitop3_b32((a), (b), (c), 0xde)
#define BITOP3_OR_NOR(a, b, c)   __builtin_amdgcn_bitop3_b32((a), (b), (c), 0xf1)

template <int NWD>
__device__ __forceinline__ void column_step_eq2(const u32 eq0, const u32 eq1, u32 (&Pv)[NWD], u32 (&Mv)[NWD])
{
    typedef unsigned long long u64;
    const u32 t0 = eq0 & Pv[0], t1 = eq1 & Pv[1];
    const u64 t = ((u64)t1 << 32) | t0, pv = ((u64)Pv[1] << 32) | Pv[0];
    u64 s;
    asm("v_lshl_add_u64 %0, %1, 0, %2" : "=v"(s) : "v"(t), "v"(pv));
    const u32 Xh0 = BITOP3_XOR_OR((u32)s, eq0, Pv[0]), Xh1 = BITOP3_XOR_OR((u32)(s >> 32), eq1, Pv[1]);
    const u32 Ph0 = BITOP3_OR_NOR(Mv[0], Xh0, Pv[0]), Ph1 = BITOP3_OR_NOR(Mv[1], Xh1, Pv[1]);
    const u32 Mh0 = Pv[0] & Xh0, Mh1 = Pv[1] & Xh1;
    u64 ph, mh;
    asm("v_lshlrev_b64 %0, 1, %1" : "=v"(ph) : "v"(((u64)Ph1 << 32) | Ph0));
    asm("v_lshlrev_b64 %0, 1, %1" : "=v"(mh) : "v"(((u64)Mh1 << 32) | Mh0));
    const u32 Xv0 = eq0 | Mv[0], Xv1 = eq1 | Mv[1];
    Pv[0] = BITOP3_OR_NOR((u32)mh, Xv0, (u32)ph);  Pv[1] = BITOP3_OR_NOR((u32)(mh >> 32), Xv1, (u32)(ph >> 32));
    Mv[0] = (u32)ph & Xv0;                          Mv[1] = (u32)(ph >> 32) & Xv1;
}

template <int NWD>
__device__ __forceinline__ void column_step_eq1(const u32 eq0, u32 (&Pv)[NWD], u32 (&Mv)[NWD])
{
    const u32 s = (eq0 & Pv[0]) + Pv[0];
    const u32 Xh = BITOP3_XOR_OR(s, eq0, Pv[0]);
    const u32 Ph = BITOP3_OR_NOR(Mv[0], Xh, Pv[0]);
    const u32 Mh = Pv[0] & Xh;
    u32 ph, mh;
    asm("v_add_u32 %0, %1, %1" : "=v"(ph) : "v"(Ph));
    asm("v_add_u32 %0, %1, %1" : "=v"(mh) : "v"(Mh));
    const u32 Xv = eq0 | Mv[0];
    Pv[0] = BITOP3_OR_NOR(mh, Xv, ph);
    Mv[0] = ph & Xv;
}

#define EDLIB_AMD_M0_EVEN(P) "s_pack_ll_b32_b16 m0, " P ", 0\n\t"
#define EDLIB_AMD_M0_ODD(P)  "s_lshr_b32 m0, " P ", 16\n\t"
#define EDLIB_AMD_RD(N, OFF) "ds_read_addtid_b32 " N " offset:" #OFF "\n\t"
#define EDLIB_AMD_RDW(N, W) "ds_read_addtid_b32 " N " offset:%[w" #W "]\n\t"

template <int NA, int W0, int CNT, int J, int S>
__device__ __forceinline__ void lds_rows_chunk(u32 (&n)[NA], const u32 pr)
{
    static_assert(CNT >= 1 && CNT <= 8 && W0 + CNT <= NA, "chunk of band words");
#define EDLIB_AMD_WOFF [w0] "n"((W0 + 0) * S * 256), [w1] "n"((W0 + 1) * S * 256), [w2] "n"((W0 + 2) * S * 256), [w3] "n"((W0 + 3) * S * 256), \
                       [w4] "n"((W0 + 4) * S * 256), [w5] "n"((W0 + 5) * S * 256), [w6] "n"((W0 + 6) * S * 256), [w7] "n"((W0 + 7) * S * 256)
#define EDLIB_AMD_ROWS_ASM(READS, OUTS)                                                                              \
    { if constexpr (J & 1) asm volatile(EDLIB_AMD_M0_ODD("%[pr]") "s_nop 0\n\t" READS : OUTS : [pr] "s"(pr), EDLIB_AMD_WOFF : "memory", "scc");   \
      else asm volatile(EDLIB_AMD_M0_EVEN("%[pr]") "s_nop 0\n\t" READS : OUTS : [pr] "s"(pr), EDLIB_AMD_WOFF : "memory", "scc"); }
#define O1 "=v"(n[W0])
#define O2 O1, "=v"(n[W0 + (CNT > 1 ? 1 : 0)])
#define O3 O2, "=v"(n[W0 + (CNT > 2 ? 2 : 0)])
#define O4 O3, "=v"(n[W0 + (CNT > 3 ? 3 : 0)])
#define O5 O4, "=v"(n[W0 + (CNT > 4 ? 4 : 0)])
#define O6 O5, "=v"(n[W0 + (CNT > 5 ? 5 : 0)])
#define O7 O6, "=v"(n[W0 + (CNT > 6 ? 6 : 0)])
#define O8 O7, "=v"(n[W0 + (CNT > 7 ? 7 : 0)])
#define R1 EDLIB_AMD_RDW("%0", 0)
#define R2 R1 EDLIB_AMD_RDW("%1", 1)
#define R3 R2 EDLIB_AMD_RDW("%2", 2)
#define R4 R3 EDLIB_AMD_RDW("%3", 3)
#define R5 R4 EDLIB_AMD_RDW("%4", 4)
#define R6 R5 EDLIB_AMD_RDW("%5", 5)
#define R7 R6 EDLIB_AMD_RDW("%6", 6)
#define R8 R7 EDLIB_AMD_RDW("%7", 7)
    if constexpr (CNT == 1) EDLIB_AMD_ROWS_ASM(R1, O1)
    if constexpr (CNT == 2) EDLIB_AMD_ROWS_ASM(R2, O2)
    if constexpr (CNT == 3) EDLIB_AMD_ROWS_ASM(R3, O3)
    if constexpr (CNT == 4) EDLIB_AMD_ROWS_ASM(R4, O4)
    if constexpr (CNT == 5) EDLIB_AMD_ROWS_ASM(R5, O5)
    if constexpr (CNT == 6) EDLIB_AMD_ROWS_ASM(R6, O6)
    if constexpr (CNT == 7) EDLIB_AMD_ROWS_ASM(R7, O7)
    if constexpr (CNT == 8) EDLIB_AMD_ROWS_ASM(R8, O8)
}
template <int NA, int J, int S>
__device__ __forceinline__ void lds_rows_request(u32 (&n)[NA], const u32 lo, const u32 hi)
{
    static_assert(NA >= 1 && NA <= 32, "band height");
    const u32 pr = (J < 2) ? lo : hi;
    lds_rows_chunk<NA, 0, (NA < 8 ? NA : 8), J, S>(n, pr);
    if constexpr (NA > 8) lds_rows_chunk<NA, 8, (NA - 8 < 8 ? NA - 8 : 8), J, S>(n, pr);
    if constexpr (NA > 16) lds_rows_chunk<NA, 16, (NA - 16 < 8 ? NA - 16 : 8), J, S>(n, pr);
    if constexpr (NA > 24) lds_rows_chunk<NA, 24, NA - 24, J, S>(n, pr);
}
template <int NA, int W0, int CNT>
__device__ __forceinline__ void lds_rows_wait_chunk(u32 (&n)[NA])
{
#define N_(i) "+v"(n[W0 + (CNT > i ? i : 0)])
    if constexpr (CNT == 1) asm volatile("s_waitcnt lgkmcnt(0)" : N_(0));
    if constexpr (CNT == 2) asm volatile("s_waitcnt lgkmcnt(0)" : N_(0), N_(1));
    if constexpr (CNT == 3) asm volatile("s_waitcnt lgkmcnt(0)" : N_(0), N_(1), N_(2));
    if constexpr (CNT == 4) asm volatile("s_waitcnt lgkmcnt(0)" : N_(0), N_(1), N_(2), N_(3));
    if constexpr (CNT == 5) asm volatile("s_waitcnt lgkmcnt(0)" : N_(0), N_(1), N_(2), N_(3), N_(4));
    if constexpr (CNT == 6) asm volatile("s_waitcnt lgkmcnt(0)" : N_(0), N_(1), N_(2), N_(3), N_(4), N_(5));
    if constexpr (CNT == 7) asm volatile("s_waitcnt lgkmcnt(0)" : N_(0), N_(1), N_(2), N_(3), N_(4), N_(5), N_(6));
    if constexpr (CNT == 8) asm volatile("s_waitcnt lgkmcnt(0)" : N_(0), N_(1), N_(2), N_(3), N_(4), N_(5), N_(6), N_(7));
#undef N_
}
template <int NA>
__device__ __forceinline__ void lds_rows_wait(u32 (&n)[NA])
{
    lds_rows_wait_chunk<NA, 0, (NA < 8 ? NA : 8)>(n);
    if constexpr (NA > 8) lds_rows_wait_chunk<NA, 8, (NA - 8 < 8 ? NA - 8 : 8)>(n);
    if constexpr (NA > 16) lds_rows_wait_chunk<NA, 16, (NA - 16 < 8 ? NA - 16 : 8)>(n);
    if constexpr (NA > 24) lds_rows_wait_chunk<NA, 24, NA - 24>(n);
}

__device__ __forceinline__ void quad_rows_request1(u32 (&n)[4], const u32 lo, const u32 hi)
{
    asm volatile(EDLIB_AMD_M0_EVEN("%[lo]") "s_nop 0\n\t" EDLIB_AMD_RD("%[n0]", 0)
                 EDLIB_AMD_M0_ODD("%[lo]") "s_nop 0\n\t" EDLIB_AMD_RD("%[n1]", 0)
                 EDLIB_AMD_M0_EVEN("%[hi]") "s_nop 0\n\t" EDLIB_AMD_RD("%[n2]", 0)
                 EDLIB_AMD_M0_ODD("%[hi]") "s_nop 0\n\t" EDLIB_AMD_RD("%[n3]", 0)
                 : [n0] "=&v"(n[0]), [n1] "=&v"(n[1]), [n2] "=&v"(n[2]), [n3] "=&v"(n[3])
                 : [lo] "s"(lo), [hi] "s"(hi) : "memory", "scc");
}
__device__ __forceinline__ void quad_rows_wait1(u32 (&n)[4]) { asm volatile("s_waitcnt lgkmcnt(0)" : "+v"(n[0]), "+v"(n[1]), "+v"(n[2]), "+v"(n[3])); }

#define EDLIB_AMD_NB_COL(C, MSET, N)                                    \
    MSET                                                                \
    "v_and_b32 %[t], " C ", %[pv]\n\t"                                  \
    EDLIB_AMD_RD(N, 0)                                                  \
    "v_add_u32 %[t], %[t], %[pv]\n\t"                                   \
    "v_bitop3_b32 %[x], %[t], " C ", %[pv] bitop3:0xde\n\t"             \
    "v_bitop3_b32 %[p], %[mv], %[x], %[pv] bitop3:0xf1\n\t"             \
    "v_and_b32 %[m], %[pv], %[x]\n\t"                                   \
    "v_add_u32 %[p], %[p], %[p]\n\t"                                    \
    "v_add_u32 %[m], %[m], %[m]\n\t"                                    \
    "v_or_b32 %[x], " C ", %[mv]\n\t"                                   \
    "v_bitop3_b32 %[pv], %[m], %[x], %[p] bitop3:0xf1\n\t"              \
    "v_and_b32 %[mv], %[p], %[x]\n\t"
__device__ __forceinline__ void quad_one_word(u32 (&c)[4], u32& Pv, u32& Mv, const u32 nlo, const u32 nhi)
{
    u32 n0, n1, n2, n3, t, x, p, m;
    asm volatile(
        EDLIB_AMD_NB_COL("%[c0]", EDLIB_AMD_M0_EVEN("%[lo]"), "%[n0]")
        EDLIB_AMD_NB_COL("%[c1]", EDLIB_AMD_M0_ODD("%[lo]"), "%[n1]")
        EDLIB_AMD_NB_COL("%[c2]", EDLIB_AMD_M0_EVEN("%[hi]"), "%[n2]")
        EDLIB_AMD_NB_COL("%[c3]", EDLIB_AMD_M0_ODD("%[hi]"), "%[n3]")
        "s_waitcnt lgkmcnt(0)"
        : [n0] "=&v"(n0), [n1] "=&v"(n1), [n2] "=&v"(n2), [n3] "=&v"(n3), [t] "=&v"(t), [x] "=&v"(x), [p] "=&v"(p), [m] "=&v"(m),
          [pv] "+v"(Pv), [mv] "+v"(Mv)
        : [c0] "v"(c[0]), [c1] "v"(c[1]), [c2] "v"(c[2]), [c3] "v"(c[3]), [lo] "s"(nlo), [hi] "s"(nhi)
        : "memory", "scc");
    c[0] = n0; c[1] = n1; c[2] = n2; c[3] = n3;
}

template <int NA, int NWD, bool CHAIN = false>
__device__ __forceinline__ void column_step_hw(const u32 (&Eq)[NA], u32 (&Pv)[NWD], u32 (&Mv)[NWD],
                                               int& e, int& flag, const u32 sh, u32& cin, u32& cout)
{
    if constexpr (!CHAIN && NWD <= 8 && NA >= 2) {
        u32 t_, s_, xh_, ph0_, ph1_, mh0_, mh1_, phs_, mhs_, xv_, Pn[NA], Mn[NA];
        unsigned long long cy_;
        if constexpr (NA == NWD) {
            int score = e, scoreN;
            RC_COLUMN_DISPATCH(NA, RC_WORD0_HW)
            e = scoreN;
            flag |= e;
        } else {
            RC_COLUMN_DISPATCH_NS(NA, RC_WORD0_HW)
        }
#pragma unroll
        for (int i = 0; i < NA; ++i) { Pv[i] = Pn[i]; Mv[i] = Mn[i]; }
        return;
    }
    u32 Ph[NA], Mh[NA];
    u32 carry = 0;
    u32 hpos = 0, hneg = 0;
    if constexpr (CHAIN) { hpos = cin & 1u; hneg = (cin >> 1) & 1u; cin >>= 2; }
#pragma unroll
    for (int i = 0; i < NA; ++i) {
        const u32 eq = (CHAIN && i == 0) ? (Eq[0] | hneg) : Eq[i];
        const u32 t = eq & Pv[i];
        u32 cout_;
        const u32 s = __builtin_addc(t, Pv[i], carry, &cout_);
        carry = cout_;
        const u32 Xh = (s ^ Pv[i]) | eq;
        Ph[i] = Mv[i] | ~(Xh | Pv[i]);
        Mh[i] = Pv[i] & Xh;
    }
    if constexpr (CHAIN) {
        const u32 x2 = (Ph[NA - 1] >> 31) | ((Mh[NA - 1] >> 30) & 2u);
        cout = __builtin_amdgcn_alignbit(x2, cout, 2);
    }
    if (NA == NWD) {
        if constexpr (NWD <= 8) {
            e += (int)((Ph[NA - 1] >> sh) & 1u);
            e -= (int)((Mh[NA - 1] >> sh) & 1u);
        } else {
            const u32 lw = sh >> 5;
            u32 phs = Ph[NWD - 1], mhs = Mh[NWD - 1];
#pragma unroll
            for (int d = 2; d <= (NWD > 16 ? 8 : 4); ++d) {
                const bool here = lw == (u32)(NWD - d);
                phs = here ? Ph[NWD - d] : phs;
                mhs = here ? Mh[NWD - d] : mhs;
            }
            e += (int)((phs >> (sh & 31u)) & 1u);
            e -= (int)((mhs >> (sh & 31u)) & 1u);
        }
        flag |= e;
    }
#pragma unroll
    for (int i = NA - 1; i >= 0; --i) {
        u32 ph, mh;
        if (i > 0) {
            ph = __builtin_amdgcn_alignbit(Ph[i], Ph[i - 1], 31);
            mh = __builtin_amdgcn_alignbit(Mh[i], Mh[i - 1], 31);
        } else if constexpr (CHAIN) {
            ph = (Ph[0] << 1) | hpos;
            mh = (Mh[0] << 1) | hneg;
        } else {
            asm("v_add_u32 %0, %1, %1" : "=v"(ph) : "v"(Ph[0]));
            asm("v_add_u32 %0, %1, %1" : "=v"(mh) : "v"(Mh[0]));
        }
        const u32 Xv = Eq[i] | Mv[i];
        Pv[i] = mh | ~(Xv | ph);
        Mv[i] = ph & Xv;
    }
}

template <int NWD> __host__ __device__ constexpr bool band_height_ok(int h)
{
    return h >= 1 && h <= NWD && (NWD <= 8 || h <= 4 || h == 6 || h == 8 || h == 12 || h == 16 || h == 24 || h == NWD);
}
template <int NWD> __host__ __device__ constexpr int band_height_up(int h)   { int n = h + 1; while (n < NWD && !band_height_ok<NWD>(n)) ++n; return n; }
template <int NWD> __host__ __device__ constexpr int band_height_down(int h) { int n = h - 1; while (n > 1 && !band_height_ok<NWD>(n)) --n; return n; }

static_assert(band_height_up<5>(3) == 4 && band_height_down<5>(3) == 2 && band_height_up<8>(7) == 8, "up to 8 words: every height");
static_assert(band_height_up<12>(4) == 6 && band_height_up<12>(8) == 12 && band_height_down<12>(12) == 8 && band_height_down<12>(6) == 4, "12-word ladder");
static_assert(band_height_up<16>(12) == 16 && band_height_down<16>(16) == 12, "16-word ladder");
static_assert(band_height_up<24>(16) == 24 && band_height_down<24>(24) == 16 && band_height_up<24>(12) == 16, "24-word ladder");
static_assert(band_height_up<32>(24) == 32 && band_height_down<32>(32) == 24 && band_height_up<32>(16) == 24, "32-word ladder");
static_assert(band_height_down<12>(12) <= 12 - 4 && band_height_down<16>(16) <= 16 - 4 && band_height_down<24>(24) <= 24 - 8 &&
              band_height_down<32>(32) <= 32 - 8, "bottom row inside the band only at full height");
static_assert(band_height_up<10>(8) == 10 && band_height_down<10>(10) <= 10 - 2 && band_height_up<14>(12) == 14 && band_height_down<14>(14) <= 14 - 2,
              "10- and 14-word ladders");

struct HwTrack {
    int best, cnt, cap;
    int* pos;
    int slot, rFirst, rLast, rMin, rPos, rCnt;
    HitList hl;
    int slotBase;

    __device__ __forceinline__ void appendRun(const bool emit) const {
        hit_list_append<4>(hl, emit, [&] { return ((unsigned long long)(u32)(slotBase + slot) << 32) | (u32)rFirst; },
                           {rLast, rMin, rPos, rCnt});
    }
};

typedef u32 QuadRows[4];

template <int NA, int NWD, int Q, int S, bool CHECK = true, bool CHAIN = false, bool FILTER = false, bool HITS = false>
__device__ __forceinline__ int band_quad(const u32 lo, const u32 hi, const u32 nlo, const u32 nhi, QuadRows& qr,
                                         const int colBase, const int colEnd, const bool track, u32 (&Pv)[NWD],
                                         u32 (&Mv)[NWD], int& e, int& flag, HwTrack& tr, const u32 sh, const int lastRows,
                                         u32& cin, u32& cout)
{
    int eh[4];
    if constexpr (NA == 1 && NWD > 1) {
        quad_one_word(qr, Pv[0], Mv[0], nlo, nhi);
    } else {
        u32 nx[NA];
        lds_rows_request<NA, 0, S>(nx, lo, hi);
#pragma unroll
        for (int j = 0; j < 4; ++j) {
            lds_rows_wait<NA>(nx);
            u32 eq[NA];
#pragma unroll
            for (int i = 0; i < NA; ++i) eq[i] = nx[i];
            if (j == 0) lds_rows_request<NA, 1, S>(nx, lo, hi);
            if (j == 1) lds_rows_request<NA, 2, S>(nx, lo, hi);
            if (j == 2) lds_rows_request<NA, 3, S>(nx, lo, hi);
            if constexpr (NA == 2 && NWD > 2) column_step_eq2<NWD>(eq[0], eq[1], Pv, Mv);
            else column_step_hw<NA, NWD, CHAIN>(eq, Pv, Mv, e, flag, sh, cin, cout);
            eh[j] = e;
        }
    }
    if (NA == NWD) {
        if (FILTER && track && __builtin_amdgcn_ballot_w64(flag < 0) != 0ull) {
            const int blk = colBase >> 4;
            bool hit = false;
#pragma unroll
            for (int j = 0; j < 4; ++j) hit = hit || (eh[j] < 0 && colBase + j < colEnd);
            bool fresh = hit;
            if (hit && tr.cnt > 0 && tr.cnt <= tr.cap) fresh = tr.pos[tr.cnt - 1] != blk;
            if (fresh && tr.cnt < tr.cap) tr.pos[tr.cnt] = blk;
            tr.cnt += fresh ? 1 : 0;
            flag = 0;
        } else if (HITS && track && __builtin_amdgcn_ballot_w64(flag < 0) != 0ull) {
#pragma unroll
            for (int j = 0; j < 4; ++j) {
                const int col = colBase + j;
                const int sc = eh[j] + tr.best + 1;
                const bool hit = eh[j] < 0 && col < colEnd && tr.cap > 0;
                const bool ext = hit && col == tr.rLast + 1, fresh = hit && !ext;
// ... 256 lines not shown
```

Baseline: 3.201 million.

## Delay bottom-row score tracking by padding rows and batch-recover scores per group

For bottom-aligned HW scans, reads are placed three rows higher in the bit vector, with padding rows that always match. The last query row's score can then be reconstructed for four consecutive columns from the top bits of Ph/Mh captured once per group. Per-column score extraction is dropped from three of every four columns, and a popcount-based group score plus a conservative threshold check triggers the detailed tracking. This adds complexity to the peq construction and kernel variants, and applies only when the longest read plus the padding rows fits in the words.

```diff
diff --git a/edlib_amd/csrc/engine.hip b/edlib_amd/csrc/engine.hip
--- a/edlib_amd/csrc/engine.hip
+++ b/edlib_amd/csrc/engine.hip
@@ -342,8 +342,8 @@
     g->nwords = w;
     g->nslots = roundup((int)units.size(), 64);
     g->perm.assign(g->nslots, -1);
-    g->mMin = 0x7fffffff;
-    for (int u : units) g->mMin = std::min(g->mMin, qlen(u));
+    g->mMin = 0x7fffffff; g->mMax = 0;
+    for (int u : units) { g->mMin = std::min(g->mMin, qlen(u)); g->mMax = std::max(g->mMax, qlen(u)); }
     std::copy(units.begin(), units.end(), g->perm.begin());
     const int nrblk = g->nslots / 64;
     if (mode == EDLIB_MODE_HW) {
diff --git a/edlib_amd/csrc/engine.hpp b/edlib_amd/csrc/engine.hpp
--- a/edlib_amd/csrc/engine.hpp
+++ b/edlib_amd/csrc/engine.hpp
@@ -197,7 +197,7 @@
     bool flatDone_ = false;
 
     struct ReadGroup {
-        int nwords = 0, nslots = 0, numSegments = 1, segLen = 0, warm = 0, mMin = 0;
+        int nwords = 0, nslots = 0, numSegments = 1, segLen = 0, warm = 0, mMin = 0, mMax = 0;
         std::vector<int> perm;
         DevBuf<int> d_perm, d_qlen, d_kinit, d_alphaExtra, d_segBest, d_segCnt, d_segPos;
         DevBuf<int> d_best, d_total, d_pos, d_flags;
@@ -253,7 +253,7 @@
                   int numSegments, int segLen, int warm, int* segBest, int* segCnt, int* segPos, int cap,
                   const long long* posOff, const int* posCap, bool unbanded = false,
                   unsigned long long* wordSteps = nullptr, const uint32_t* peqDense = nullptr,
-                  const int* qlenDense = nullptr, bool peqBottom = false);
+                  const int* qlenDense = nullptr, int peqBottom = 0);
 
     DevBuf<PairDesc> d_descs_;
     DevBuf<unsigned long long> d_peq64_;
diff --git a/edlib_amd/csrc/engine_reads.hip b/edlib_amd/csrc/engine_reads.hip
--- a/edlib_amd/csrc/engine_reads.hip
+++ b/edlib_amd/csrc/engine_reads.hip
@@ -21,7 +21,7 @@
 int Batch::scanGroup(ReadGroup& g, int mode, const int* d_slotmap, int nlanes, int kcap, const int* d_kinit,
                      int numSegments, int segLen, int warm, int* segBest, int* segCnt, int* segPos, int cap,
                      const long long* posOff, const int* posCap, bool unbanded, unsigned long long* wordSteps,
-                     const uint32_t* peqDense, const int* qlenDense, bool peqBottom)
+                     const uint32_t* peqDense, const int* qlenDense, int peqBottom)
 {
     ReadScanArgs a{};
     a.peq = peqDense ? peqDense : g.d_peq.p; a.tpk = d_tpk_.p; a.trows = d_trows_.p; a.targetLength = tlen(0);
@@ -32,15 +32,16 @@
     a.posOff = posOff; a.posCap = posCap;
     a.kcap = kcap; a.wordSteps = wordSteps ? wordSteps : d_wordSteps_.p;
     a.filter = filterScan_ ? 1 : 0;
-    a.bottomAligned = peqBottom ? 1 : 0;
+    a.bottomAligned = peqBottom;
     a.chainIn = chain_.in; a.chainOut = chain_.out; a.chainSrc = chain_.src; a.chainInLanes = chain_.inLanes;
     a.chainBlocks = chain_.blocks; a.rowBase = chain_.rowBase;
     const bool chained = chain_.in != nullptr || chain_.out != nullptr;
     static const bool dbg = getenv("EDLIB_AMD_DEBUG") != nullptr;
     if (dbg) {
         EDLIB_AMD_HIP(hipStreamSynchronize(stream_));
-        fprintf(stderr, "[edlib_amd] scanGroup nwords=%d mode=%d nlanes=%d S=%d segLen=%d warm=%d cap=%d kcap=%d slotmap=%p posOff=%p\n",
-                g.nwords, mode, nlanes, numSegments, segLen, warm, cap, kcap, (const void*)d_slotmap, (const void*)posOff);
+        fprintf(stderr, "[edlib_amd] scanGroup nwords=%d mode=%d nlanes=%d S=%d segLen=%d warm=%d cap=%d kcap=%d slotmap=%p posOff=%p rows=%s\n",
+                g.nwords, mode, nlanes, numSegments, segLen, warm, cap, kcap, (const void*)d_slotmap, (const void*)posOff,
+                peqBottom > 1 ? "delay" : (peqBottom ? "bottom" : "top"));
     }
     scanTimerStart();
     const bool longGroup = g.nwords > kMaxReadWords;
@@ -251,8 +252,9 @@
                 plain = (double)ws >= 0.85 * g.nwords * cols;
                 stats.word_steps += (long long)ws;
             }
-            const bool bottom = plain && mode == EDLIB_MODE_HW && syms_ == 4 && g.nwords <= kMaxReadWords &&
-                                chain_.in == nullptr && chain_.out == nullptr;
+            const bool bottomOk = plain && mode == EDLIB_MODE_HW && syms_ == 4 && g.nwords <= kMaxReadWords &&
+                                  chain_.in == nullptr && chain_.out == nullptr;
+            const int bottom = !bottomOk ? 0 : (delay_rows_fit(g.nwords, g.mMax) ? 1 + kDelayRows : 1);
             const size_t no64 = (no + 63) / 64 * 64;
             std::vector<int> perm2(no64, -1);
             for (size_t i = 0; i < no; ++i) perm2[i] = g.perm[todo[i]];
diff --git a/edlib_amd/csrc/reads_column_asm.hpp b/edlib_amd/csrc/reads_column_asm.hpp
--- a/edlib_amd/csrc/reads_column_asm.hpp
+++ b/edlib_amd/csrc/reads_column_asm.hpp
@@ -88,13 +88,13 @@
 #define RP_SCORE(PH, MH)   "v_lshrrev_b32_e64 %[t], 31, " PH "\n\t" "v_add_u32_e64 %[scoreN], %[score], %[t]\n\t" \
                            "v_ashrrev_i32_e64 %[t], 31, " MH "\n\t" "v_add_u32_e64 %[scoreN], %[scoreN], %[t]\n\t"
 #define RP_PAIR01          RP_S1_0(RP_P0, RP_M0) RP_S1(1, RP_P1, RP_M1)
-#define RP_BODY_2 RP_PAIR01 RP_SCORE(RP_P1, RP_M1) RP_SHL RP_S2(0, RP_P0, RP_M0) RP_S2(1, RP_P1, RP_M1)
-#define RP_BODY_3 RP_PAIR01 RP_S1(2, RP_PL, RP_ML) RP_SCORE(RP_PL, RP_ML) RP_LONE RP_SHL \
+#define RP_BODY_2(SC) RP_PAIR01 SC(RP_P1, RP_M1) RP_SHL RP_S2(0, RP_P0, RP_M0) RP_S2(1, RP_P1, RP_M1)
+#define RP_BODY_3(SC) RP_PAIR01 RP_S1(2, RP_PL, RP_ML) SC(RP_PL, RP_ML) RP_LONE RP_SHL \
                   RP_S2(0, RP_P0, RP_M0) RP_S2(1, RP_P1, RP_M1) RP_S2(2, RP_PL, RP_ML)
-#define RP_BODY_4 RP_PAIR01 RP_CARRY RP_SHL RP_S2(0, RP_P0, RP_M0) RP_S2(1, RP_P1, RP_M1) \
-                  RP_S1(2, RP_P0, RP_M0) RP_S1(3, RP_P1, RP_M1) RP_SCORE(RP_P1, RP_M1) RP_SHLADD RP_S2(2, RP_P0, RP_M0) RP_S2(3, RP_P1, RP_M1)
-#define RP_BODY_5 RP_PAIR01 RP_CARRY RP_SHL RP_S2(0, RP_P0, RP_M0) RP_S2(1, RP_P1, RP_M1) \
-                  RP_S1(2, RP_P0, RP_M0) RP_S1(3, RP_P1, RP_M1) RP_S1(4, RP_PL, RP_ML) RP_SCORE(RP_PL, RP_ML) RP_LONE RP_SHLADD \
+#define RP_BODY_4(SC) RP_PAIR01 RP_CARRY RP_SHL RP_S2(0, RP_P0, RP_M0) RP_S2(1, RP_P1, RP_M1) \
+                  RP_S1(2, RP_P0, RP_M0) RP_S1(3, RP_P1, RP_M1) SC(RP_P1, RP_M1) RP_SHLADD RP_S2(2, RP_P0, RP_M0) RP_S2(3, RP_P1, RP_M1)
+#define RP_BODY_5(SC) RP_PAIR01 RP_CARRY RP_SHL RP_S2(0, RP_P0, RP_M0) RP_S2(1, RP_P1, RP_M1) \
+                  RP_S1(2, RP_P0, RP_M0) RP_S1(3, RP_P1, RP_M1) RP_S1(4, RP_PL, RP_ML) SC(RP_PL, RP_ML) RP_LONE RP_SHLADD \
                   RP_S2(2, RP_P0, RP_M0) RP_S2(3, RP_P1, RP_M1) RP_S2(4, RP_PL, RP_ML)
 #define RP_TEMPS [t] "=&v"(t_), [ph0] "=&{v56}"(ph0_), [ph1] "=&{v57}"(ph1_), [mh0] "=&{v58}"(mh0_), [mh1] "=&{v59}"(mh1_), [cy] "=&s"(cy_)
 #define RP_TEMPS_LONE , [phl] "=&v"(phl_), [mhl] "=&v"(mhl_)
@@ -108,7 +108,7 @@
 #define RP_XI_4 RP_INS_CARRY
 #define RP_XT_5 RP_TEMPS_LONE RP_TEMPS_CARRY
 #define RP_XI_5 RP_INS_CARRY
-#define RP_COLUMN_ASM_B(N) asm(RC_HEAD RP_BODY_##N : RC_OUTS_##N, [scoreN] "=&v"(scoreN), RP_TEMPS RP_XT_##N : RC_INS_##N, [score] "v"(score) RP_XI_##N)
+#define RP_COLUMN_ASM_B(N) asm(RC_HEAD RP_BODY_##N(RP_SCORE) : RC_OUTS_##N, [scoreN] "=&v"(scoreN), RP_TEMPS RP_XT_##N : RC_INS_##N, [score] "v"(score) RP_XI_##N)
 #define RP_COLUMN_DISPATCH_B(NWD) \
     if constexpr (NWD == 2) RP_COLUMN_ASM_B(2); if constexpr (NWD == 3) RP_COLUMN_ASM_B(3); \
     if constexpr (NWD == 4) RP_COLUMN_ASM_B(4); if constexpr (NWD == 5) RP_COLUMN_ASM_B(5);
@@ -117,6 +117,29 @@
     if constexpr (NA == 1) RC_COLUMN_ASM_NS(1, WORD0); if constexpr (NA == 2) RC_COLUMN_ASM_NS(2, WORD0); if constexpr (NA == 3) RC_COLUMN_ASM_NS(3, WORD0); \
     if constexpr (NA == 4) RC_COLUMN_ASM_NS(4, WORD0); if constexpr (NA == 5) RC_COLUMN_ASM_NS(5, WORD0); if constexpr (NA == 6) RC_COLUMN_ASM_NS(6, WORD0); \
     if constexpr (NA == 7) RC_COLUMN_ASM_NS(7, WORD0); if constexpr (NA == 8) RC_COLUMN_ASM_NS(8, WORD0);
+#define RP_SC_NONE(PH, MH)
+#define RP_SC_CAPTURE(PH, MH) "v_lshrrev_b32_e64 %[nph], 28, " PH "\n\t" "v_lshrrev_b32_e64 %[nmh], 28, " MH "\n\t" RC_GROUP_UPDATE
+#define RP_SC_BIT28(PH, MH)   "v_bfe_u32 %[t], " PH ", 28, 1\n\t" "v_add_u32_e64 %[scoreN], %[score], %[t]\n\t" \
+                              "v_bfe_i32 %[t], " MH ", 28, 1\n\t" "v_add_u32_e64 %[scoreN], %[scoreN], %[t]\n\t"
+#define RP_COLUMN_ASM_D0(N) asm(RC_HEAD RP_BODY_##N(RP_SC_NONE) : RC_OUTS_##N, RP_TEMPS RP_XT_##N : RC_INS_##N RP_XI_##N)
+#define RC_GROUP_UPDATE "v_bcnt_u32_b32 %[scoreN], %[nph], %[score]\n\t" "v_bcnt_u32_b32 %[t], %[nmh], 0\n\t" \
+                        "v_sub_u32_e64 %[scoreN], %[scoreN], %[t]\n\t"
+#define RC_GROUP_OUTS [nph] "=&v"(nph), [nmh] "=&v"(nmh), [scoreN] "=&v"(scoreN)
+#define RP_COLUMN_ASM_D1(N) asm(RC_HEAD RP_BODY_##N(RP_SC_CAPTURE) : RC_OUTS_##N, RC_GROUP_OUTS, RP_TEMPS RP_XT_##N : RC_INS_##N, [score] "v"(score) RP_XI_##N)
+#define RP_COLUMN_ASM_D2(N) asm(RC_HEAD RP_BODY_##N(RP_SC_BIT28) : RC_OUTS_##N, [scoreN] "=&v"(scoreN), RP_TEMPS RP_XT_##N : RC_INS_##N, [score] "v"(score) RP_XI_##N)
+#define RP_COLUMN_DISPATCH_D(F, NWD) \
+    if constexpr (NWD == 2) RP_COLUMN_ASM_D##F(2); if constexpr (NWD == 3) RP_COLUMN_ASM_D##F(3); \
+    if constexpr (NWD == 4) RP_COLUMN_ASM_D##F(4); if constexpr (NWD == 5) RP_COLUMN_ASM_D##F(5);
+#define RC_SC_CAPTURE(c)  "v_lshrrev_b32_e64 %[nph], 28, %[ph" #c "]\n\t" "v_lshrrev_b32_e64 %[nmh], 28, %[mh" #c "]\n\t"
+#define RC_SC_BIT28(c)    "v_bfe_u32 %[t], %[ph" #c "], 28, 1\n\t" "v_bfe_i32 %[s], %[mh" #c "], 28, 1\n\t" "v_add3_u32 %[scoreN], %[score], %[t], %[s]\n\t"
+#define RC_SC_CAPTURE_X(c) RC_SC_CAPTURE(c)
+#define RC_SC_BIT28_X(c) RC_SC_BIT28(c)
+#define RC_COLUMN_ASM_D0(N) RC_COLUMN_ASM_NS(N, RC_WORD0_HW)
+#define RC_COLUMN_ASM_D1(N) asm(RC_HEAD RC_WORD0_HW RC_REST_##N RC_SC_CAPTURE_X(RC_LAST_##N) RC_GROUP_UPDATE : RC_OUTS_##N, RC_GROUP_OUTS, RC_TEMPS : RC_INS_##N, [score] "v"(score))
+#define RC_COLUMN_ASM_D2(N) asm(RC_HEAD RC_WORD0_HW RC_REST_##N RC_SC_BIT28_X(RC_LAST_##N) : RC_OUTS_##N, [scoreN] "=&v"(scoreN), RC_TEMPS : RC_INS_##N, [score] "v"(score))
+#define RC_COLUMN_DISPATCH_D(F, NWD) \
+    if constexpr (NWD == 1) RC_COLUMN_ASM_D##F(1); if constexpr (NWD == 6) RC_COLUMN_ASM_D##F(6); \
+    if constexpr (NWD == 7) RC_COLUMN_ASM_D##F(7); if constexpr (NWD == 8) RC_COLUMN_ASM_D##F(8);
 #define RC_COLUMN_DISPATCH_B(NWD, WORD0) \
     if constexpr (NWD == 1) RC_COLUMN_ASM_B(1, WORD0); if constexpr (NWD == 2) RC_COLUMN_ASM_B(2, WORD0); if constexpr (NWD == 3) RC_COLUMN_ASM_B(3, WORD0); \
     if constexpr (NWD == 4) RC_COLUMN_ASM_B(4, WORD0); if constexpr (NWD == 5) RC_COLUMN_ASM_B(5, WORD0); if constexpr (NWD == 6) RC_COLUMN_ASM_B(6, WORD0); \
diff --git a/edlib_amd/csrc/reads_kernels.hip b/edlib_amd/csrc/reads_kernels.hip
--- a/edlib_amd/csrc/reads_kernels.hip
+++ b/edlib_amd/csrc/reads_kernels.hip
@@ -97,13 +97,14 @@
             unsigned long long seen0 = 0, seen1 = 0, seen2 = 0, seen3 = 0;
             int extraJ = 0;
             const bool mine = lane == j;
-            const int padj = bottomAlign ? 32 * NWD - mj : 0;
+            const int delay = bottomAlign > 1 ? bottomAlign - 1 : 0;
+            const int padj = bottomAlign ? 32 * NWD - delay - mj : 0;
 #pragma unroll
             for (int c = 0; c < (NWD + 1) / 2; ++c) {
                 const int i = 64 * c + lane - padj;
                 const bool in = i >= 0 && i < mj;
                 const u32 by = in ? reads[offj + i] : 0u;
-                const u32 mask = in ? ((u32)s_eq[by] >> g0) : (i < 0 ? 0xfu : 0u);
+                const u32 mask = in ? ((u32)s_eq[by] >> g0) : ((i < 0 || i < mj + delay) ? 0xfu : 0u);
                 const unsigned long long b0 = __builtin_amdgcn_ballot_w64((mask & 1u) != 0), b1 = __builtin_amdgcn_ballot_w64((mask & 2u) != 0);
                 const unsigned long long b2 = __builtin_amdgcn_ballot_w64((mask & 4u) != 0), b3 = __builtin_amdgcn_ballot_w64((mask & 8u) != 0);
                 constexpr int w0 = 0;
@@ -146,19 +147,20 @@
 static hipError_t launch_build_peq_t(const uint8_t* reads, const long long* qoff, const int* perm,
                                      int nslots, int S, const uint16_t* eqtbl, const u32* tpres, int kcfg,
                                      u32* peq, int* qlen, int* kinit, int* alphaExtra,
-                                     hipStream_t stream, bool bottomAlign)
+                                     hipStream_t stream, int bottomAlign)
 {
     hipLaunchKernelGGL(build_peq_reads_kernel<NWD>, dim3((nslots + 255) / 256), dim3(256), 0, stream,
-                       reads, qoff, perm, nslots, S, eqtbl, tpres, kcfg, peq, qlen, kinit, alphaExtra, bottomAlign ? 1 : 0);
+                       reads, qoff, perm, nslots, S, eqtbl, tpres, kcfg, peq, qlen, kinit, alphaExtra, bottomAlign);
     return hipGetLastError();
 }
 
 hipError_t launch_build_peq_reads(int nwords, int syms, const uint8_t* reads, const long long* qoff,
                                   const int* perm, int nslots, const uint16_t* eqtbl,
                                   const u32* tpres, int kcfg, u32* peq, int* qlen, int* kinit,
-                                  int* alphaExtra, hipStream_t stream, bool bottomAlign)
+                                  int* alphaExtra, hipStream_t stream, int bottomAlign)
 {
     if (nslots == 0) return hipSuccess;
+    if (bottomAlign != 0 && bottomAlign != 1 && bottomAlign != 1 + kDelayRows) return hipErrorInvalidValue;
     if (syms != 4 && syms != 8 && syms != 16) return hipErrorInvalidValue;
     switch (nwords) {
 #define CASE(N) case N: return launch_build_peq_t<N>(reads, qoff, perm, nslots, syms, eqtbl, tpres, kcfg, peq, qlen, kinit, alphaExtra, stream, bottomAlign);
@@ -177,6 +179,14 @@
         default: column_step<NWD, MODE, BOTTOM>(E3, Pv, Mv, score, sh, zr0, zr1); asm volatile("; sym3"); break; \
     }
 
+#define EDLIB_AMD_DISPATCH_COLUMN_DELAY(FORM, sym)                                         \
+    switch (sym) {                                                                         \
+        case 0:  column_step_delay<NWD, FORM>(E0, Pv, Mv, score, nph, nmh, zr0, zr1); asm volatile("; sym0"); break; \
+        case 1:  column_step_delay<NWD, FORM>(E1, Pv, Mv, score, nph, nmh, zr0, zr1); asm volatile("; sym1"); break; \
+        case 2:  column_step_delay<NWD, FORM>(E2, Pv, Mv, score, nph, nmh, zr0, zr1); asm volatile("; sym2"); break; \
+        default: column_step_delay<NWD, FORM>(E3, Pv, Mv, score, nph, nmh, zr0, zr1); asm volatile("; sym3"); break; \
+    }
+
 #define EDLIB_AMD_TRACK_SCORE(sc, col)                         \
     if ((sc) <= best) {                                        \
         if ((sc) < best) { best = (sc); cnt = 0; }             \
@@ -185,11 +195,13 @@
     }
 #define EDLIB_AMD_TRACK(col) EDLIB_AMD_TRACK_SCORE(score, col)
 
-template <int NWD, int MODE, bool BOTTOM = false>
+template <int NWD, int MODE, bool BOTTOM = false, bool DELAY = false>
 __global__ void __launch_bounds__(256)
 scan_reads_kernel(const ReadScanArgs a)
 {
+    static_assert(!DELAY || (BOTTOM && MODE == 2), "delay rows: bottom-aligned HW rows");
     constexpr int kHitGroup = 4;
+    static_assert(!DELAY || kHitGroup == kDelayRows + 1, "one nibble per group");
     const int lane = threadIdx.x & 63;
     const int rblk = blockIdx.x * 4 + (threadIdx.x >> 6);
     const int seg = blockIdx.y;
@@ -213,7 +225,7 @@
     }
     const int m = a.qlen[slot];
     if constexpr (BOTTOM) {
-        const int pad = 32 * NWD - m;
+        const int pad = 32 * NWD - (DELAY ? kDelayRows : 0) - m;
 #pragma unroll
         for (int d = 0; d < NWD; ++d) {
             const int lo = pad - 32 * d;
@@ -239,17 +251,59 @@
     int cw = c0 - a.warm; if (cw < 0) cw = 0;
     cw &= ~15;
 
+    u32 nph = 0, nmh = 0;
     for (int w = cw >> 4; w < (c0 >> 4); ++w) {
         const u32 tw = a.tpk[w];
 #pragma unroll
         for (int j = 0; j < 16; ++j) {
             const u32 sym = (tw >> (2 * j)) & 3u;
-            EDLIB_AMD_DISPATCH_COLUMN(sym)
+            if constexpr (!DELAY) {
+                EDLIB_AMD_DISPATCH_COLUMN(sym)
+            } else if ((j & (kHitGroup - 1)) != kHitGroup - 1) {
+                EDLIB_AMD_DISPATCH_COLUMN_DELAY(0, sym)
+            } else {
+                EDLIB_AMD_DISPATCH_COLUMN_DELAY(1, sym)
+            }
         }
     }
     const int wend = c1 >> 4;
     int lim = best + (kHitGroup - 1);
-    for (int w = c0 >> 4; w < wend; ++w) {
+    if constexpr (DELAY) {
+        int lim2 = 2 * best + kHitGroup;
+        for (int w = c0 >> 4; w < wend; ++w) {
+            const u32 tw = a.tpk[w];
+#pragma unroll
+            for (int j = 0; j < 16; j += kHitGroup) {
+#pragma unroll
+                for (int q = 0; q < kHitGroup - 1; ++q) {
+                    const u32 sym = (tw >> (2 * (j + q))) & 3u;
+                    EDLIB_AMD_DISPATCH_COLUMN_DELAY(0, sym)
+                }
+                const int before = score;
+                {
+                    const u32 sym = (tw >> (2 * (j + kHitGroup - 1))) & 3u;
+                    EDLIB_AMD_DISPATCH_COLUMN_DELAY(1, sym)
+                }
+                if (__builtin_expect(score + before <= lim2, 0)) {
+                    int sc[kHitGroup], acc = before, least = 0x7fffffff;
+#pragma unroll
+                    for (int q = 0; q < kHitGroup; ++q) {
+                        acc += (int)((nph >> (kHitGroup - 1 - q)) & 1u) - (int)((nmh >> (kHitGroup - 1 - q)) & 1u);
+                        sc[q] = acc;
+                        least = acc < least ? acc : least;
+                    }
+                    best = (lim2 - kHitGroup) >> 1;
+                    if (least <= best) {
+#pragma unroll
+                        for (int q = 0; q < kHitGroup; ++q) { EDLIB_AMD_TRACK_SCORE(sc[q], w * 16 + j + q) }
+                        lim2 = 2 * best + kHitGroup;
+                    }
+                }
+            }
+        }
+        lim = ((lim2 - kHitGroup) >> 1) + (kHitGroup - 1);
+    }
+    for (int w = c0 >> 4; !DELAY && w < wend; ++w) {
         const u32 tw = a.tpk[w];
 #pragma unroll
         for (int j = 0; j < 16; j += kHitGroup) {
@@ -277,7 +331,7 @@
         for (int j = 0; j < rem; ++j) {
             const u32 sym = tw & 3u;
             tw >>= 2;
-            EDLIB_AMD_DISPATCH_COLUMN(sym)
+            if constexpr (DELAY) { EDLIB_AMD_DISPATCH_COLUMN_DELAY(2, sym) } else { EDLIB_AMD_DISPATCH_COLUMN(sym) }
             if (MODE != 0) { EDLIB_AMD_TRACK(wend * 16 + j) }
         }
     }
@@ -296,7 +350,8 @@
     switch (mode) {
         case 0: hipLaunchKernelGGL((scan_reads_kernel<NWD, 0>), grid, block, 0, stream, a); break;
         case 1: hipLaunchKernelGGL((scan_reads_kernel<NWD, 1>), grid, block, 0, stream, a); break;
-        case 2: if (a.bottomAligned) hipLaunchKernelGGL((scan_reads_kernel<NWD, 2, true>), grid, block, 0, stream, a);
+        case 2: if (a.bottomAligned == 1 + kDelayRows) hipLaunchKernelGGL((scan_reads_kernel<NWD, 2, true, true>), grid, block, 0, stream, a);
+                else if (a.bottomAligned) hipLaunchKernelGGL((scan_reads_kernel<NWD, 2, true>), grid, block, 0, stream, a);
                 else hipLaunchKernelGGL((scan_reads_kernel<NWD, 2>), grid, block, 0, stream, a);
                 break;
         default: return hipErrorInvalidValue;
@@ -308,6 +363,7 @@
 {
     if (a.nlanes == 0) return hipSuccess;
     if (a.bottomAligned && mode != 2) return hipErrorInvalidValue;
+    if (a.bottomAligned != 0 && a.bottomAligned != 1 && a.bottomAligned != 1 + kDelayRows) return hipErrorInvalidValue;
     switch (nwords) {
 #define CASE(N) case N: return launch_scan_mode<N>(mode, a, stream);
         CASE(1) CASE(2) CASE(3) CASE(4) CASE(5) CASE(6) CASE(7) CASE(8)
diff --git a/edlib_amd/csrc/reads_kernels.hpp b/edlib_amd/csrc/reads_kernels.hpp
--- a/edlib_amd/csrc/reads_kernels.hpp
+++ b/edlib_amd/csrc/reads_kernels.hpp
@@ -11,6 +11,8 @@
 constexpr int kMaxLongReadWords4 = 32;
 constexpr int kFilterFromWords = 13;
 inline int read_group_words(int m) { const int w = (m + 31) / 32; return w <= kMaxReadWords ? w : (w <= 10 ? 10 : (w <= 12 ? 12 : (w <= 14 ? 14 : (w <= 16 ? 16 : (w <= 24 ? 24 : 32))))); }
+constexpr int kDelayRows = 3;
+constexpr bool delay_rows_fit(int nwords, int longest) { return nwords <= kMaxReadWords && longest >= 1 && longest + kDelayRows <= 32 * nwords; }
 constexpr int kLanes = 64;
 
 
@@ -60,7 +62,7 @@
                                   const int* perm, int nslots, const uint16_t* eqtbl,
                                   const uint32_t* targetPresence , int kcfg,
                                   uint32_t* peq, int* qlen, int* kinit, int* alphaExtra,
-                                  hipStream_t stream, bool bottomAlign = false);
+                                  hipStream_t stream, int bottomAlign = 0);
 
 hipError_t launch_collect_candidates(const int* segCnt, const int* segPos, int numSegments, int cap, int nlanes,
                                      int* out, int maxOut, int* counter, int* overflow, hipStream_t stream);
diff --git a/edlib_amd/csrc/reads_scan.hpp b/edlib_amd/csrc/reads_scan.hpp
--- a/edlib_amd/csrc/reads_scan.hpp
+++ b/edlib_amd/csrc/reads_scan.hpp
@@ -68,6 +68,30 @@
         Pv[i] = mh | ~(Xv | ph);
         Mv[i] = ph & Xv;
     }
+}
+
+template <int NWD, int FORM>
+__device__ __forceinline__ void column_step_delay(const u32 (&Eq)[NWD], u32 (&Pv)[NWD], u32 (&Mv)[NWD],
+                                                  int& score, u32& nph, u32& nmh, const u32 zr0, const u32 zr1)
+{
+    static_assert(NWD >= 1 && NWD <= 8 && FORM >= 0 && FORM <= 2, "delay rows: up to 8 words");
+    u32 Pn[NWD], Mn[NWD];
+    int scoreN = score;
+    unsigned long long cy_;
+    if constexpr (NWD >= 2 && NWD <= 5) {
+        u32 t_, ph0_, ph1_, mh0_, mh1_, phl_, mhl_, cp_, cm_;
+        if constexpr (FORM == 0) { RP_COLUMN_DISPATCH_D(0, NWD) }
+        if constexpr (FORM == 1) { RP_COLUMN_DISPATCH_D(1, NWD) }
+        if constexpr (FORM == 2) { RP_COLUMN_DISPATCH_D(2, NWD) }
+    } else {
+        u32 t_, s_, xh_, ph0_, ph1_, mh0_, mh1_, phs_, mhs_, xv_;
+        if constexpr (FORM == 0) { RC_COLUMN_DISPATCH_D(0, NWD) }
+        if constexpr (FORM == 1) { RC_COLUMN_DISPATCH_D(1, NWD) }
+        if constexpr (FORM == 2) { RC_COLUMN_DISPATCH_D(2, NWD) }
+    }
+#pragma unroll
+    for (int i = 0; i < NWD; ++i) { Pv[i] = Pn[i]; Mv[i] = Mn[i]; }
+    score = scoreN;
 }
 
 
```

After: 3.273 million, median of 6. +2.2%, better.
